# mariohsouto/ProxSDP.jl

Hardware: AMD Instinct MI355X
Metric: PDHG iterations/sec at target rank ~ sqrt(n), Max-Cut SDP n=4000 (tol 1e-4 options) (higher is better)
Workload: dtype f64

## Files before the change

### include/proxsdp_hip.h

```cpp
#ifndef PROXSDP_HIP_H
#define PROXSDP_HIP_H

#include <stdint.h>

#ifdef __cplusplus
extern "C" {
#endif

#define PROXSDP_HIP_ABI_VERSION 10

#define PROXSDP_E_INVALID  (-1)
#define PROXSDP_E_HIP      (-2)
#define PROXSDP_E_NOMEM    (-3)
#define PROXSDP_E_UNSUPP   (-4)
#define PROXSDP_E_INTERNAL (-5)
#define PROXSDP_E_COMM_ABORTED (-6)

#define PROXSDP_STATUS_NOT_CALLED       0
#define PROXSDP_STATUS_OPTIMAL          1
#define PROXSDP_STATUS_TIME_LIMIT       2
#define PROXSDP_STATUS_ITERATION_LIMIT  3
#define PROXSDP_STATUS_INFEAS_OR_UNBND  4
#define PROXSDP_STATUS_DUAL_INFEASIBLE  5
#define PROXSDP_STATUS_INFEASIBLE       6
// ... 29 lines not shown
    const double* M_dense;
    int32_t M_dense_on_device;
    int32_t reserved1;
    int64_t n_coupling;
    const int64_t* coupling_rows;
    const int32_t* coupling_owned;
    int (*reduce_vec_fn)(void* ctx, double* buf, int64_t len, int32_t on_device);
    int32_t reduce_vec_on_device;
    int32_t reserved2;
    void* nccl_comm;
    int64_t reserved3;
} proxsdp_problem;

typedef struct proxsdp_options {
    int64_t struct_size;
    int32_t log_verbose;  int32_t log_freq;
    int32_t timer_verbose; int32_t timer_file; int32_t disable_julia_logger;
    int32_t warn_on_limit; int32_t extended_log; int32_t extended_log2; int32_t log_repeat_header;
    int32_t pad0;
    double  time_limit;
    double tol_gap, tol_feasibility, tol_feasibility_dual, tol_primal, tol_dual, tol_psd, tol_soc;
    int32_t check_dual_feas; int32_t check_dual_feas_freq;
    double  max_obj; int32_t min_iter_max_obj; int32_t pad1;
    int32_t min_iter_time_infeas; int32_t pad2;
    double infeas_gap_tol, infeas_limit_gap_tol, infeas_stable_gap_tol,
           infeas_feasibility_tol, infeas_stable_feasibility_tol;
    int32_t certificate_search; int32_t pad3;
    double certificate_obj_tol, certificate_fail_tol;
    double min_beta, max_beta, initial_beta;
    double initial_adapt_level, adapt_decay; int32_t adapt_window; int32_t pad4;
    int32_t convergence_window; int32_t convergence_check;
    int64_t max_iter; int64_t min_iter; int64_t divergence_min_update;
    int64_t max_iter_lp; int64_t max_iter_conic; int64_t max_iter_local;
    int32_t advanced_initialization; int32_t line_search_flag;
    int32_t max_linsearch_steps; int32_t pad5;
    double delta, initial_theta, linsearch_decay;
    int32_t full_eig_decomp; int32_t max_target_rank_krylov_eigs;
    int32_t min_size_krylov_eigs; int32_t warm_start_eig;
    int32_t rank_increment; int32_t rank_increment_factor;
    int32_t eigsolver; int32_t eigsolver_min_lanczos; int64_t eigsolver_resid_seed;
    double  arpack_tol; int32_t arpack_resid_init; int32_t arpack_reset_resid; int64_t arpack_max_iter;
    int32_t krylovkit_reset_resid; int32_t krylovkit_resid_init;
    double  krylovkit_tol; int32_t krylovkit_max_iter; int32_t krylovkit_eager; int32_t krylovkit_verbose;
    int32_t reduce_rank; int32_t rank_slack; int32_t pad6;
    int64_t full_eig_freq; int64_t full_eig_len;
    int32_t equilibration; int32_t equilibration_iters;
    double  equilibration_lb, equilibration_ub, equilibration_limit;
    int32_t equilibration_force; int32_t approx_norm;
    int32_t device_id;
    int32_t trace_capacity;
    int32_t profile_symv_every;
    int32_t support_path;
    int32_t lanczos_operator;
    int32_t initial_target_rank;
    int32_t full_eig_lanczos;
    int32_t lanczos_cycle_kernel;
    int32_t lanczos_warm_start;
    int32_t reconstruct_mfma;
    int32_t small_block_batch;
    int32_t full_eig_sign;
    int32_t psd_sign_engine;
    int32_t full_eig_lanczos_verify;
    double  full_eig_lanczos_posres;
    int32_t full_eig_lanczos_kdim10;
    int32_t sign_small_tile_max;
    int32_t host_eig_threads;
    int32_t block_threads;
    int32_t host_eig_merge;
    int32_t block_batch;
    int32_t rocsolver_warmup;
    int32_t debug_fail_iteration;
    int32_t host_wait_spin;
    int32_t sign_start_row;
    int32_t general_batch;
    int32_t full_eig_lanczos_certify;
    int32_t host_merge_threads;
    int32_t reserved_i[1];
    double  full_eig_lanczos_tol;
    double  reserved_d[1];
    int32_t equilibration_reference_aliasing;
    int32_t reserved_i3[2];
    int32_t block_batch_groups;
    int32_t lanczos_wide_krylov;
    int32_t reserved_i2[7];
    double  full_eig_lanczos_warm_pow;
    double  reserved_d2[3];
} proxsdp_options;

#define PROXSDP_TRACE_COLS 14

typedef struct proxsdp_stats {
    int64_t lanczos_matvecs;
    int64_t lanczos_restarts;
    int64_t lanczos_calls;
    int64_t full_eigs;
    int64_t krylov_fallbacks;
    int64_t linesearch_trials;
    int64_t symv_launches;
    int64_t symv_profiled;
    double  symv_profiled_ms;
    double  symv_bytes;
    double  algorithmic_bytes;
    double  init_time;
    double  loop_time;
    double  exit_time;
    double  t_primal, t_psd, t_linesearch, t_residual;
    int64_t dense_passes;
    double  dense_ms;
    int64_t fop_projections;
    int64_t exit_matvecs;
    double  host_eig_time;
    int64_t host_eigs;
    int64_t device_eigs;
    int64_t batched_small_eigs;
    int64_t mfma_reconstructions;
    int64_t orth_profiled;
    double  orth_profiled_ms;
    double  full_eig_solver_ms;
    double  full_eig_recon_ms;
    int64_t cycle_launches;
    int64_t full_eigs_lanczos;
    int64_t cycle_steps;
    double  cycle_ms;
    int64_t warm_starts;
    int64_t full_eigs_sign;
    int64_t sign_products;
    int64_t sign_engine_projections;
    int64_t sign_engine_rejected;
    int64_t sign_engine_checks;
    int64_t sign_engine_mismatches;
    int64_t full_eigs_lanczos_checks;
    int64_t full_eigs_lanczos_mismatches;
    int64_t batched_block_steps;
    int64_t rccl_reductions;
    int64_t batched_profiled_blocks;
    int64_t host_eig_merges;
    double  host_eig_overlap_time;
    int64_t sign_short_pass;
    int64_t sign_short_fail;
    int64_t full_eigs_lanczos_certified;
    int64_t full_eigs_lanczos_cert_failed;
    int64_t cert_matvecs;
    int64_t dense_truncated_projections;
    int64_t wide_krylov_projections;
    int64_t reserved_s[4];
    int64_t dense_setup_passes;
    int64_t dense_sigma_steps;
} proxsdp_stats;
#define PROXSDP_STATS_SHARDED_GENERAL_ITERATIONS 0

typedef struct proxsdp_result {
    int32_t status;
    int32_t certificate_found;
    int32_t primal_feasible_user_tol;
    int32_t dual_feasible_user_tol;
    int32_t result_count;
    int32_t final_rank;
    int64_t iter;
    double  primal_residual;
    double  dual_residual;
    double  objval, dual_objval, gap, time;
    double  dual_feasibility;
    double* primal;
    double* dual_cone;
    double* dual_eq;
    double* dual_in;
    double* slack_eq;
    double* slack_in;
    double* trace;
    int64_t trace_rows;
    char    status_string[256];
    proxsdp_stats stats;
} proxsdp_result;

#define PROXSDP_STATE_NHIST 7
typedef struct proxsdp_state {
    int64_t struct_size;
    int64_t iteration;
    int64_t n, Q, n_psd;
    int64_t hist_len;
    double* x;
    double* y;
    double* Mty;
    double* Mx;
    int64_t* target_rank;
    int64_t* current_rank;
    double* min_eig;
    double* hist;
    double scal[16];
    int64_t ints[8];
} proxsdp_state;

int  proxsdp_hip_abi_version(void);
void proxsdp_hip_default_options(proxsdp_options* opt);
int  proxsdp_hip_set_option(proxsdp_options* opt, const char* name, double value);
int  proxsdp_hip_get_option(const proxsdp_options* opt, const char* name, double* value);
int  proxsdp_hip_solve(const proxsdp_problem* prob, const proxsdp_options* opt,
                       proxsdp_result* res);
int  proxsdp_hip_solve_ex(const proxsdp_problem* prob, const proxsdp_options* opt, proxsdp_result* res,
                          const proxsdp_state* resume, proxsdp_state* capture);
const char* proxsdp_hip_last_error(void);
int  proxsdp_hip_device_count(void);

int  proxsdp_hip_solve_sharded(const proxsdp_problem* prob, const proxsdp_options* opt,
                               int32_t n_shards, const int32_t* device_ids,
                               const int32_t* psd_owner, const int32_t* soc_owner, const int32_t* free_owner,
                               proxsdp_result* res, proxsdp_stats* shard_stats);

#define PROXSDP_FACTOR_NONE 0
#define PROXSDP_FACTOR_RITZ 1
#define PROXSDP_FACTOR_EIG  2
typedef struct proxsdp_psd_factors {
    int64_t struct_size;
    int64_t n_psd;
    const int64_t* cap;
    const int64_t* vec_ptr;
    const int64_t* val_ptr;
    double*  vectors;
    double*  values;
    int64_t* rank;
    int64_t* rank_found;
    int32_t* source;
    double*  resid;
    double*  xnorm;
} proxsdp_psd_factors;
int  proxsdp_hip_solve_factored(const proxsdp_problem* prob, const proxsdp_options* opt, proxsdp_result* res,
                                proxsdp_psd_factors* fac);

typedef struct proxsdp_start {
    int64_t struct_size;
    const double* primal;
    const double* dual_eq;
// ... 54 lines not shown
int proxsdp_hip_dual_trial(const double* y, const double* Mx, const double* Mx_old, const double* bh,
                           int64_t p, int64_t Q, double bt, double theta, double* y_out, double* ynorm2);

int proxsdp_hip_residuals(const double* x, const double* x_old, const double* Mty, const double* Mty_old,
                          const double* c, double tau, int64_t n,
                          const double* y, const double* y_old, const double* Mx, const double* Mx_old,
                          const double* bh, int64_t p, int64_t Q, double sigma, double* out);

typedef struct {
    int64_t struct_size;
    int64_t p;
    const double* bh; const double* y; const double* Mx; const double* Mx_old;
    const double* x; const double* x_old; const double* Mty_old;
    const double* roww;
    double xold_coef, tau_update;
    int32_t support, nc, plain, c0;
    double tau[3], theta[3], bt[3], sigma[3];
    double tau_re, sigma_re;
    double* y_out;
    double* Mty_out;
    double* scal;
    double* scal_re;
    int32_t* supp_out;
    double* x_upd; double* xsave; double* esv;
    int64_t ns;
    int32_t gq, gx;
} proxsdp_trial_batch;
int proxsdp_hip_trial_batch(const proxsdp_csc* M, int32_t index_base, const double* c, proxsdp_trial_batch* t);

int proxsdp_hip_cone_tail(const double* x, int64_t n, const int64_t* soc_off, const int32_t* soc_len, int32_t nsoc,
                          const int64_t* one_off, int32_t n_one, double* x_soc, double* gap_in, double* gap_out,
                          double* x_clamp, double* min_eig);

typedef struct {
    int64_t struct_size;
    int32_t n, tile, epilogue, use_dsc;
    const double* P; const double* Q; const double* Y;
    double ca, cb, cc;
    double dsc[3];
    const double* xold;
    const uint32_t* mask; int64_t mask_words, mask_off;
    double sentinel;
    double* T;
    double* part;
    double* xp;
    double* respart;
    int32_t ld, grid;
} proxsdp_sym_product;
int proxsdp_hip_sym_product(proxsdp_sym_product* t);

int proxsdp_hip_sign_unpack(const double* packed, int64_t n, double sentinel, double* A, double* sc);

int proxsdp_hip_dense_scaling(const proxsdp_problem* prob, const proxsdp_options* opt,
                              double* E, double* D, double* frob, double* sigma_max, int32_t* equilibrated);

int proxsdp_hip_coupling_sum(const double* parts, int32_t n_shards, int64_t len, const int64_t* rows,
                             const double* v_in, int64_t n, double* v_out);

typedef struct proxsdp_shard {
    int64_t struct_size;
    int64_t n, p, m, nnz_A, nnz_G, n_coupling, n_psd, len_psd, n_soc, len_soc, len_eig;
    int64_t* vars; int64_t* rows_eq; int64_t* rows_in;
    int64_t* coupling_rows; int32_t* coupling_owned;
    int64_t* A_colptr; int64_t* A_rowval; double* A_nzval;
    int64_t* G_colptr; int64_t* G_rowval; double* G_nzval;
    double* b; double* h; double* c;
    int64_t* psd_ids; int64_t* psd_ptr; int64_t* psd_idx;
    int64_t* soc_ids; int64_t* soc_ptr; int64_t* soc_idx;
    double* eig_resid;
} proxsdp_shard;
int proxsdp_host_split_shard(const proxsdp_problem* prob, int32_t n_shards, const int32_t* psd_owner,
                             const int32_t* soc_owner, const int32_t* free_owner, int32_t shard, proxsdp_shard* out);
int proxsdp_host_group_reduce(int32_t n_shards, int32_t rounds, int32_t nsum, int32_t nmax, const double* records,
                              int32_t leave_shard, int32_t leave_after, double timeout_s,
                              double* out, int32_t* rounds_done, int32_t* failed);
int proxsdp_host_symeig(int32_t k, double* a, double* d);
int proxsdp_host_symeig_threads(int32_t k, double* a, double* d, int32_t threads);
int proxsdp_host_symeig_arrow(int32_t K, int32_t m, const double* D, const double* f,
                              const double* al, const double* be, double* U, double* d);
int proxsdp_host_symeig_split(int32_t K, int32_t m, int32_t k1, const double* D, const double* f,
                              const double* al, const double* be, double* U, double* d, int32_t* info);
int proxsdp_host_symeig_split_threads(int32_t K, int32_t m, int32_t k1, const double* D, const double* f,
                                      const double* al, const double* be, int32_t threads, double* U, double* d, int32_t* info);
int proxsdp_host_start_vector(int64_t n, int64_t seed, int32_t init, double* out);
int proxsdp_host_preprocess(const proxsdp_problem* prob, int64_t* order, int64_t* var_ordering,
                            double* c_scaled, double* frobenius_norm_M);
int proxsdp_host_equilibrate_rowsums(const double* rowsums, int64_t Q, int64_t n, const proxsdp_options* opt,
                                     double* E, double* d);

#ifdef __cplusplus
}
#endif
#endif
```

### proxsdp.jl_amd/binding.py

```python
import ctypes as C
import os
import pathlib
import re

import numpy as np
import scipy.sparse as sp

_HERE = pathlib.Path(__file__).resolve().parent
LIB_PATH = _HERE / "libproxsdp_hip.so"
HEADER_PATH = _HERE.parent / "include" / "proxsdp_hip.h"

TRACE_COLS = 14
TRACE_NAMES = ("iter", "prim_obj", "dual_obj", "gap", "feas", "prim_res", "dual_res",
               "primal_step", "beta", "theta", "target_rank", "trials", "elapsed", "matvecs")


class LibraryNotBuilt(RuntimeError):
    pass


class ProxSDPHipError(RuntimeError):
    def __init__(self, code, msg):
        super().__init__(f"libproxsdp_hip error {code}: {msg}")
        self.code = code


i32, i64, f64 = C.c_int32, C.c_int64, C.c_double
pi64 = C.POINTER(C.c_int64)
pf64 = C.POINTER(C.c_double)


class CSC(C.Structure):
    _fields_ = [("nrows", i64), ("ncols", i64), ("colptr", pi64), ("rowval", pi64), ("nzval", pf64)]


class Problem(C.Structure):
    _fields_ = [("n", i64), ("p", i64), ("m", i64), ("A", CSC), ("G", CSC),
                ("b", pf64), ("h", pf64), ("c", pf64),
                ("n_psd", i64), ("psd_ptr", pi64), ("psd_idx", pi64),
                ("n_soc", i64), ("soc_ptr", pi64), ("soc_idx", pi64),
                ("index_base", i32), ("reserved0", i32), ("eig_resid", pf64),
                ("reduce_ctx", C.c_void_p), ("reduce_fn", C.c_void_p),
                ("M_dense", C.c_void_p), ("M_dense_on_device", i32), ("reserved1", i32),
                ("n_coupling", i64), ("coupling_rows", pi64), ("coupling_owned", C.POINTER(i32)),
                ("reduce_vec_fn", C.c_void_p), ("reduce_vec_on_device", i32), ("reserved2", i32),
                ("nccl_comm", C.c_void_p), ("reserved3", i64)]


REDUCE_FN = C.CFUNCTYPE(C.c_int, C.c_void_p, pf64, i32, pf64, i32)
REDUCE_VEC_FN = C.CFUNCTYPE(C.c_int, C.c_void_p, C.c_void_p, i64, i32)


def _opt_fields():
    F = []
    a = lambda name, t: F.append((name, t))
    a("struct_size", i64)
    for nme in ("log_verbose", "log_freq", "timer_verbose", "timer_file", "disable_julia_logger",
                "warn_on_limit", "extended_log", "extended_log2", "log_repeat_header", "pad0"):
        a(nme, i32)
    a("time_limit", f64)
    for nme in ("tol_gap", "tol_feasibility", "tol_feasibility_dual", "tol_primal", "tol_dual",
                "tol_psd", "tol_soc"):
        a(nme, f64)
    a("check_dual_feas", i32); a("check_dual_feas_freq", i32)
    a("max_obj", f64); a("min_iter_max_obj", i32); a("pad1", i32)
    a("min_iter_time_infeas", i32); a("pad2", i32)
    for nme in ("infeas_gap_tol", "infeas_limit_gap_tol", "infeas_stable_gap_tol",
                "infeas_feasibility_tol", "infeas_stable_feasibility_tol"):
        a(nme, f64)
    a("certificate_search", i32); a("pad3", i32)
    a("certificate_obj_tol", f64); a("certificate_fail_tol", f64)
    a("min_beta", f64); a("max_beta", f64); a("initial_beta", f64)
    a("initial_adapt_level", f64); a("adapt_decay", f64); a("adapt_window", i32); a("pad4", i32)
    a("convergence_window", i32); a("convergence_check", i32)
    for nme in ("max_iter", "min_iter", "divergence_min_update", "max_iter_lp", "max_iter_conic",
                "max_iter_local"):
        a(nme, i64)
    a("advanced_initialization", i32); a("line_search_flag", i32)
    a("max_linsearch_steps", i32); a("pad5", i32)
    a("delta", f64); a("initial_theta", f64); a("linsearch_decay", f64)
    a("full_eig_decomp", i32); a("max_target_rank_krylov_eigs", i32)
    a("min_size_krylov_eigs", i32); a("warm_start_eig", i32)
    a("rank_increment", i32); a("rank_increment_factor", i32)
    a("eigsolver", i32); a("eigsolver_min_lanczos", i32); a("eigsolver_resid_seed", i64)
    a("arpack_tol", f64); a("arpack_resid_init", i32); a("arpack_reset_resid", i32); a("arpack_max_iter", i64)
    a("krylovkit_reset_resid", i32); a("krylovkit_resid_init", i32)
    a("krylovkit_tol", f64); a("krylovkit_max_iter", i32); a("krylovkit_eager", i32); a("krylovkit_verbose", i32)
    a("reduce_rank", i32); a("rank_slack", i32); a("pad6", i32)
    a("full_eig_freq", i64); a("full_eig_len", i64)
    a("equilibration", i32); a("equilibration_iters", i32)
    a("equilibration_lb", f64); a("equilibration_ub", f64); a("equilibration_limit", f64)
    a("equilibration_force", i32); a("approx_norm", i32)
    a("device_id", i32); a("trace_capacity", i32); a("profile_symv_every", i32); a("support_path", i32)
    a("lanczos_operator", i32); a("initial_target_rank", i32)
    a("full_eig_lanczos", i32); a("lanczos_cycle_kernel", i32); a("lanczos_warm_start", i32)
    a("reconstruct_mfma", i32); a("small_block_batch", i32); a("full_eig_sign", i32); a("psd_sign_engine", i32)
    a("full_eig_lanczos_verify", i32); a("full_eig_lanczos_posres", f64); a("full_eig_lanczos_kdim10", i32)
    a("sign_small_tile_max", i32); a("host_eig_threads", i32); a("block_threads", i32)
    a("host_eig_merge", i32); a("block_batch", i32); a("rocsolver_warmup", i32); a("debug_fail_iteration", i32); a("host_wait_spin", i32)
    a("sign_start_row", i32); a("general_batch", i32); a("full_eig_lanczos_certify", i32); a("host_merge_threads", i32); a("reserved_i", i32 * 1)
    a("full_eig_lanczos_tol", f64); a("reserved_d", f64 * 1)
    a("equilibration_reference_aliasing", i32); a("reserved_i3", i32 * 2)
    a("block_batch_groups", i32); a("lanczos_wide_krylov", i32); a("reserved_i2", i32 * 7); a("full_eig_lanczos_warm_pow", f64); a("reserved_d2", f64 * 3)
    return F


class Options(C.Structure):
    _fields_ = _opt_fields()


class Stats(C.Structure):
    _fields_ = [("lanczos_matvecs", i64), ("lanczos_restarts", i64), ("lanczos_calls", i64),
                ("full_eigs", i64), ("krylov_fallbacks", i64), ("linesearch_trials", i64),
                ("symv_launches", i64), ("symv_profiled", i64), ("symv_profiled_ms", f64),
                ("symv_bytes", f64), ("algorithmic_bytes", f64), ("init_time", f64),
                ("loop_time", f64), ("exit_time", f64), ("t_primal", f64), ("t_psd", f64),
                ("t_linesearch", f64), ("t_residual", f64), ("dense_passes", i64), ("dense_ms", f64), ("fop_projections", i64), ("exit_matvecs", i64),
                ("host_eig_time", f64), ("host_eigs", i64), ("device_eigs", i64), ("batched_small_eigs", i64),
                ("mfma_reconstructions", i64), ("orth_profiled", i64), ("orth_profiled_ms", f64),
                ("full_eig_solver_ms", f64), ("full_eig_recon_ms", f64), ("cycle_launches", i64),
                ("full_eigs_lanczos", i64), ("cycle_steps", i64), ("cycle_ms", f64), ("warm_starts", i64),
                ("full_eigs_sign", i64), ("sign_products", i64),
                ("sign_engine_projections", i64), ("sign_engine_rejected", i64),
                ("sign_engine_checks", i64), ("sign_engine_mismatches", i64),
                ("full_eigs_lanczos_checks", i64), ("full_eigs_lanczos_mismatches", i64),
                ("batched_block_steps", i64), ("rccl_reductions", i64),
                ("batched_profiled_blocks", i64), ("host_eig_merges", i64),
                ("host_eig_overlap_time", f64), ("sign_short_pass", i64), ("sign_short_fail", i64),
                ("full_eigs_lanczos_certified", i64), ("full_eigs_lanczos_cert_failed", i64), ("cert_matvecs", i64),
                ("dense_truncated_projections", i64), ("wide_krylov_projections", i64), ("reserved_s", i64 * 4),
                ("dense_setup_passes", i64), ("dense_sigma_steps", i64)]


class Result(C.Structure):
    _fields_ = [("status", i32), ("certificate_found", i32), ("primal_feasible_user_tol", i32),
                ("dual_feasible_user_tol", i32), ("result_count", i32), ("final_rank", i32),
                ("iter", i64), ("primal_residual", f64), ("dual_residual", f64),
                ("objval", f64), ("dual_objval", f64), ("gap", f64), ("time", f64),
                ("dual_feasibility", f64),
                ("primal", pf64), ("dual_cone", pf64), ("dual_eq", pf64), ("dual_in", pf64),
                ("slack_eq", pf64), ("slack_in", pf64), ("trace", pf64), ("trace_rows", i64),
                ("status_string", C.c_char * 256), ("stats", Stats)]


STATS_RESERVED_SLOTS = {"sharded_general_iterations": 0}

STATE_NHIST = 7
STATE_HIST_NAMES = ("dual_gap", "prim_obj", "dual_obj", "feasibility", "primal_residual", "dual_residual", "comb_residual")
STATE_SCAL_NAMES = ("primal_step", "primal_step_old", "dual_step", "beta", "theta", "adapt_level",
                    "equa_feasibility", "ineq_feasibility", "dual_feasibility")


class State(C.Structure):
    _fields_ = [("struct_size", i64), ("iteration", i64), ("n", i64), ("Q", i64), ("n_psd", i64), ("hist_len", i64),
                ("x", pf64), ("y", pf64), ("Mty", pf64), ("Mx", pf64),
                ("target_rank", pi64), ("current_rank", pi64), ("min_eig", pf64), ("hist", pf64),
                ("scal", f64 * 16), ("ints", i64 * 8)]


class ShardIO(C.Structure):
    _fields_ = ([("struct_size", i64)] +
                [(k, i64) for k in ("n", "p", "m", "nnz_A", "nnz_G", "n_coupling", "n_psd", "len_psd", "n_soc", "len_soc", "len_eig")] +
                [("vars", pi64), ("rows_eq", pi64), ("rows_in", pi64), ("coupling_rows", pi64), ("coupling_owned", C.POINTER(i32)),
                 ("A_colptr", pi64), ("A_rowval", pi64), ("A_nzval", pf64), ("G_colptr", pi64), ("G_rowval", pi64), ("G_nzval", pf64),
                 ("b", pf64), ("h", pf64), ("c", pf64),
                 ("psd_ids", pi64), ("psd_ptr", pi64), ("psd_idx", pi64), ("soc_ids", pi64), ("soc_ptr", pi64), ("soc_idx", pi64), ("eig_resid", pf64)])


class PsdFactors(C.Structure):
    _fields_ = [("struct_size", i64), ("n_psd", i64), ("cap", pi64), ("vec_ptr", pi64), ("val_ptr", pi64),
                ("vectors", pf64), ("values", pf64), ("rank", pi64), ("rank_found", pi64), ("source", C.POINTER(i32)),
                ("resid", pf64), ("xnorm", pf64)]


class Start(C.Structure):
    _fields_ = [("struct_size", i64), ("primal", pf64), ("dual_eq", pf64), ("dual_in", pf64), ("n_psd", i64),
                ("rank", pi64), ("vec_ptr", pi64), ("val_ptr", pi64), ("vectors", pf64), ("values", pf64),
                ("target_rank", pi64), ("primal_step", f64), ("beta", f64)]


FACTOR_NONE, FACTOR_RITZ, FACTOR_EIG = 0, 1, 2
FACTOR_SOURCE_NAMES = {FACTOR_NONE: "NONE", FACTOR_RITZ: "RITZ", FACTOR_EIG: "EIG"}


_lib = None


def header_symbols():
    txt = HEADER_PATH.read_text()
    txt = re.sub(r"/\*.*?\*/", "", txt, flags=re.S)
    return sorted(set(re.findall(r"\b(proxsdp_(?:hip|host)_\w+)\s*\(", txt)))


def lib():
    global _lib
    if _lib is not None:
        return _lib
    if not LIB_PATH.exists():
        raise LibraryNotBuilt(
            f"{LIB_PATH} is missing: run `python -c 'import __graft_entry__ as g; g.build()'` "
            "(or `make -C proxsdp.jl_amd/csrc`).  There is no CPU fallback.")
    import sys
    if "torch" in sys.modules:
        try:
            tc = sys.modules["torch"].cuda
            if tc.is_available():
                tc.init()
        except Exception:
            pass
    L = C.CDLL(str(LIB_PATH))
    L.proxsdp_hip_abi_version.restype = C.c_int
    L.proxsdp_hip_last_error.restype = C.c_char_p
    L.proxsdp_hip_default_options.argtypes = [C.POINTER(Options)]
    L.proxsdp_hip_default_options.restype = None
    L.proxsdp_hip_set_option.argtypes = [C.POINTER(Options), C.c_char_p, f64]
    L.proxsdp_hip_get_option.argtypes = [C.POINTER(Options), C.c_char_p, pf64]
    L.proxsdp_hip_solve.argtypes = [C.POINTER(Problem), C.POINTER(Options), C.POINTER(Result)]
    L.proxsdp_hip_solve_ex.argtypes = [C.POINTER(Problem), C.POINTER(Options), C.POINTER(Result),
                                       C.POINTER(State), C.POINTER(State)]
    L.proxsdp_hip_solve_factored.argtypes = [C.POINTER(Problem), C.POINTER(Options), C.POINTER(Result),
                                             C.POINTER(PsdFactors)]
    L.proxsdp_hip_solve_from.argtypes = [C.POINTER(Problem), C.POINTER(Options), C.POINTER(Result),
                                         C.POINTER(Start), C.POINTER(PsdFactors)]
    L.proxsdp_hip_start_point.argtypes = [C.POINTER(Problem), C.POINTER(Options), C.POINTER(Start), C.POINTER(State)]
    L.proxsdp_hip_factor_residual.argtypes = [pf64, i64, pf64, i64, pf64, i32, pf64, pf64]
    L.proxsdp_hip_factor_residual_kernel.argtypes = [pf64, i64, pf64, i64, pf64, i32, pf64, pf64, i32, pf64]
    L.proxsdp_hip_psd_project.argtypes = [pf64, i64, i32, i32, C.POINTER(Options), pf64, pf64,
                                          C.POINTER(i32), pf64, pi64, C.POINTER(i32), C.POINTER(i32)]
# ... 778 lines not shown
    if epi < 2:
        out["T"] = np.zeros((ld, ld), order="F")
        t.T = _p(out["T"])
    else:
        out["xp"] = np.zeros(N)
        t.xp = _p(out["xp"])
    if want_part or epi >= 2:
        part = np.zeros(cap)
        t.part = _p(part)
    if epi == 3:
        xo = _f(xold)
        mk = np.ascontiguousarray(mask, dtype=np.uint32)
        assert len(xo) == N
        t.xold, t.mask, t.mask_words, t.mask_off = _p(xo), _p(mk, C.POINTER(C.c_uint32)), len(mk), int(mask_off)
        resp = np.zeros(2 * cap)
        t.respart = _p(resp)
    _check(lib().proxsdp_hip_sym_product(C.byref(t)))
    assert t.ld == ld and t.grid <= cap
    out.update(ld=ld, grid=int(t.grid), part=part[:t.grid].copy() if (want_part or epi >= 2) else None)
    if epi == 3:
        out["respart"] = resp[:2 * t.grid].reshape(2, t.grid).copy()
    return out


def sign_unpack(packed, n, sentinel=SYM_SENTINEL):
    xin = _f(packed)
    assert len(xin) == n * (n + 1) // 2
    ld = 64 * ((n + 63) // 64)
    A = np.zeros((ld, ld), order="F")
    sc = np.zeros(16)
    _check(lib().proxsdp_hip_sign_unpack(_p(xin), n, float(sentinel), _p(A), _p(sc)))
    return A, sc


def dense_scaling(prob, options=None):
    M = _Marshalled(prob)
    Q = M.P.p + M.P.m
    E, D = np.zeros(max(Q, 1)), np.zeros(max(M.P.n, 1))
    fro, sig, eq = f64(), f64(), i32()
    _check(lib().proxsdp_hip_dense_scaling(C.byref(M.P), C.byref(options) if options is not None else None,
                                           _p(E), _p(D), C.byref(fro), C.byref(sig), C.byref(eq)))
    return E[:Q], D[:M.P.n], fro.value, sig.value, bool(eq.value)


def host_symeig(A, threads=-1):
    L = lib()
    a = np.asfortranarray(A, dtype=np.float64).copy(order="F")
    k = a.shape[0]
    d = np.zeros(k)
    _check(L.proxsdp_host_symeig_threads(k, a.ctypes.data_as(pf64), _p(d), threads))
    return d, a


def host_symeig_arrow(D, f, al, be):
    L = lib()
    D, f, al, be = _f(D), _f(f), _f(al), _f(be)
    K, m = len(al), len(D)
    U = np.zeros((K, K), order="F")
    d = np.zeros(K)
    L.proxsdp_host_symeig_arrow.argtypes = [i32, i32, pf64, pf64, pf64, pf64, pf64, pf64]
    _check(L.proxsdp_host_symeig_arrow(K, m, _p(D), _p(f), _p(al), _p(be), U.ctypes.data_as(pf64), _p(d)))
    return d, U


def host_start_vector(n, seed=1234, init=3):
    out = np.zeros(n)
    _check(lib().proxsdp_host_start_vector(n, seed, init, _p(out)))
    return out


def host_symeig_split(D, f, al, be, k1, threads=0):
    D = _f(D); f = _f(f); al = _f(al); be = _f(be)
    K, m = len(al), len(D)
    U = np.zeros((K, K))
    d = np.zeros(K)
    info = (i32 * 3)()
    L = lib()
    L.proxsdp_host_symeig_split_threads.argtypes = [i32, i32, i32, pf64, pf64, pf64, pf64, i32, pf64, pf64, C.POINTER(i32)]
    _check(L.proxsdp_host_symeig_split_threads(K, m, int(k1), _p(D) if m else None, _p(f) if m else None, _p(al), _p(be),
                                               int(threads), _p(U), _p(d), info))
    return d, U.T.copy(), dict(nondeflated=info[0], deflated=info[1], max_secular_iterations=info[2])


def host_preprocess(prob, index_base=0):
    M = _Marshalled(prob, index_base=index_base)
    n = prob.n
    order, inv = np.zeros(n, dtype=np.int64), np.zeros(n, dtype=np.int64)
    cs = np.zeros(n)
    fro = f64()
    _check(lib().proxsdp_host_preprocess(C.byref(M.P), _p(order, pi64), _p(inv, pi64), _p(cs), C.byref(fro)))
    return order, inv, cs, fro.value


def host_equilibrate_rowsums(rowsums, n, options=None):
    rs = _f(rowsums)
    E = np.zeros(max(len(rs), 1))
    d = f64()
    _check(lib().proxsdp_host_equilibrate_rowsums(_p(rs), len(rs), int(n), C.byref(options) if options is not None else None,
                                                  _p(E), C.byref(d)))
    return E[:len(rs)], d.value
```

### proxsdp.jl_amd/csrc/capi.hip

```cpp
#include <functional>
#include <memory>
#include <new>
#include <string>

#include "pdhg_loop.hip.hpp"
#include "projection.hip.hpp"
#include "shard_split.hpp"

namespace {
thread_local std::string g_last_error;

template <typename F>
int guarded(F&& f) {
    try {
        g_last_error.clear();
        return f();
    } catch (const std::bad_alloc&) {
        g_last_error = "out of memory";
        return PROXSDP_E_NOMEM;
    } catch (const proxsdp::HipError& e) {
        g_last_error = e.what();
        return PROXSDP_E_HIP;
    } catch (const std::invalid_argument& e) {
        g_last_error = e.what();
// ... 853 lines not shown
    return guarded([&]() -> int {
        if (n <= 0 || Q <= 0 || p < 0 || p > Q || !x || !x_old || !Mty || !Mty_old || !c || !y || !y_old || !Mx ||
            !Mx_old || !bh || !out) throw std::invalid_argument("invalid argument");
        Engine E(nullptr, 2, 2);
        hipStream_t st = E.S.stream;
        using proxsdp::DevBuf;
        const int gx = std::min(proxsdp::PSTRIDE, proxsdp::grid_for(n)), gq = std::min(proxsdp::PSTRIDE, proxsdp::grid_for(Q));
        DevBuf<double> dx(n), dxo(n), dm(n), dmo(n), dc(n), dy(Q), dyo(Q), d1(Q), d0(Q), dbh(Q);
        DevBuf<double> part((size_t)11 * proxsdp::PSTRIDE), sc(9);
        dx.upload(x, n, st); dxo.upload(x_old, n, st); dm.upload(Mty, n, st); dmo.upload(Mty_old, n, st); dc.upload(c, n, st);
        dy.upload(y, Q, st); dyo.upload(y_old, Q, st); d1.upload(Mx, Q, st); d0.upload(Mx_old, Q, st); dbh.upload(bh, Q, st);
        part.zero(st);
        proxsdp::dev::TrialBatch tb{};
        tb.nc = 1; tb.tau[0] = tau; tb.sigma[0] = sigma;
        hipLaunchKernelGGL(proxsdp::dev::k_residual_xy<false>, dim3(std::max(gx, gq), 1, 2), dim3(proxsdp::dev::TPB), 0, st,
                           (const double*)dx.p, (const int*)nullptr, (long long)n, (const double*)dxo.p, 1.0,
                           (const double*)dm.p, (long long)n, (const double*)dmo.p, (const double*)dc.p, gx,
                           (const double*)dy.p, (long long)Q, (const double*)dyo.p, (const double*)d1.p, (const double*)d0.p,
                           (const double*)dbh.p, (int)p, (int)Q, gq, tb, part.p, proxsdp::PSTRIDE, 0LL, (const double*)nullptr);
        hipLaunchKernelGGL(proxsdp::dev::k_combine_multi, dim3(3), dim3(proxsdp::dev::TPB), 0, st,
                           (const double*)(part.p + (size_t)2 * proxsdp::PSTRIDE), proxsdp::PSTRIDE, gx, 0x3ull, sc.p, 3,
                           (const double*)nullptr, 0, 0, (double*)nullptr);
        hipLaunchKernelGGL(proxsdp::dev::k_combine_multi, dim3(6), dim3(proxsdp::dev::TPB), 0, st,
                           (const double*)(part.p + (size_t)5 * proxsdp::PSTRIDE), proxsdp::PSTRIDE, gq, 0xFull, sc.p + 3, 6,
                           (const double*)nullptr, 0, 0, (double*)nullptr);
        sc.download(out, 9, st);
        PX_HIP(hipStreamSynchronize(st));
        return 0;
    });
}

int proxsdp_host_symeig(int32_t k, double* a, double* d) {
    return proxsdp_host_symeig_threads(k, a, d, -1);
}

int proxsdp_host_symeig_threads(int32_t k, double* a, double* d, int32_t threads) {
    if (k < 0 || !a || !d) { g_last_error = "invalid argument"; return PROXSDP_E_INVALID; }
    int rc = proxsdp::symeig_dense(k, a, d, false, threads);
    if (rc != 0) { g_last_error = "QL iteration did not converge"; return PROXSDP_E_INTERNAL; }
    return 0;
}

int proxsdp_host_symeig_arrow(int32_t K, int32_t m, const double* D, const double* f,
                              const double* al, const double* be, double* U, double* d) {
    if (K < 2 || m < 1 || m >= K || !D || !f || !al || !be || !U || !d) { g_last_error = "invalid argument"; return PROXSDP_E_INVALID; }
    const int n1 = m + 1;
    std::vector<double> Qa((size_t)n1 * n1, 0.0), da(n1), ea(n1);
    for (int j = 0; j < m; ++j) { Qa[(size_t)j * n1 + j] = D[j]; Qa[(size_t)j * n1 + m] = Qa[(size_t)m * n1 + j] = f[j]; }
    proxsdp::householder_tridiag(n1, Qa.data(), da.data(), ea.data());
    int rc = proxsdp::symeig_tridiag_from(K, m, Qa.data(), da.data(), ea.data(), al, be, U, d);
    if (rc != 0) { g_last_error = "QL iteration did not converge"; return PROXSDP_E_INTERNAL; }
    return 0;
}

int proxsdp_host_symeig_split(int32_t K, int32_t m, int32_t k1, const double* D, const double* f,
                              const double* al, const double* be, double* U, double* d, int32_t* info) {
    return proxsdp_host_symeig_split_threads(K, m, k1, D, f, al, be, 0, U, d, info);
}

int proxsdp_host_symeig_split_threads(int32_t K, int32_t m, int32_t k1, const double* D, const double* f,
                                      const double* al, const double* be, int32_t threads, double* U, double* d, int32_t* info) {
    return guarded([&]() -> int {
        if (K < 2 || m < 0 || m >= K || k1 < 1 || k1 >= K || !al || !be || !U || !d) throw std::invalid_argument("invalid argument");
        proxsdp::SplitEig S;
        std::unique_ptr<proxsdp::SpinPool> pool;
        proxsdp::ParFor par;
        struct Guard { proxsdp::SpinPool* p; ~Guard() { if (p) p->disarm(); } } guard{nullptr};
        if (threads > 0) {
            pool.reset(new proxsdp::SpinPool(std::min<int>(threads, 15)));
            pool->arm();
            guard.p = pool.get();
            par = [&pool](int n, const std::function<void(int)>& body) { pool->run(n, body); };
            S.M.par = &par;
            S.M.nchunk = std::min<int>(threads, 15) + 1;
        }
        if (S.first(k1, m, D, f, al, be) != 0 || S.second(K, al, be) != 0) throw std::invalid_argument("split eigensolver failed");
        std::vector<int> cols(K);
        for (int c = 0; c < K; ++c) { cols[c] = c; d[c] = S.M.evals[c]; }
        S.M.vectors(cols.data(), K, U);
        if (info) { info[0] = S.M.k; info[1] = (int)S.M.df.size(); info[2] = S.M.max_iter_seen; }
        return 0;
    });
}
int proxsdp_host_start_vector(int64_t n, int64_t seed, int32_t init, double* out) {
    if (n < 0 || !out) { g_last_error = "invalid argument"; return PROXSDP_E_INVALID; }
    proxsdp::start_vector(n, (uint64_t)seed, init, out);
    return 0;
}

int proxsdp_host_preprocess(const proxsdp_problem* prob, int64_t* order, int64_t* var_ordering,
                            double* c_scaled, double* frobenius_norm_M) {
    return guarded([&]() -> int {
        if (!prob) throw std::invalid_argument("NULL problem");
        proxsdp::Prep R = proxsdp::prepare(*prob, nullptr, prob->reduce_fn != nullptr || prob->nccl_comm != nullptr);
        for (int64_t i = 0; i < R.n; ++i) {
            if (order) order[i] = R.ord[i];
            if (var_ordering) var_ordering[i] = R.inv[i];
            if (c_scaled) c_scaled[i] = R.c[i];
        }
        if (frobenius_norm_M) *frobenius_norm_M = R.frob;
        return 0;
    });
}

int proxsdp_host_split_shard(const proxsdp_problem* prob, int32_t n_shards, const int32_t* psd_owner,
                             const int32_t* soc_owner, const int32_t* free_owner, int32_t shard, proxsdp_shard* out) {
    return guarded([&]() -> int {
        if (!prob || !out) throw std::invalid_argument("NULL problem or output");
        if (out->struct_size != (int64_t)sizeof(proxsdp_shard)) throw std::invalid_argument("proxsdp_shard.struct_size mismatch");
        const proxsdp::ShardPlan L = proxsdp::plan_shards(*prob, n_shards, psd_owner, soc_owner, free_owner);
        if (shard < 0 || shard >= n_shards) throw std::invalid_argument("shard outside 0 .. n_shards - 1");
        const proxsdp::ShardData S = proxsdp::split_shard(*prob, L, shard);
        out->n = (int64_t)S.vars.size(); out->p = (int64_t)S.rows_eq.size(); out->m = (int64_t)S.rows_in.size();
        out->nnz_A = (int64_t)S.A_rowval.size(); out->nnz_G = (int64_t)S.G_rowval.size();
        out->n_coupling = (int64_t)S.coup_rows.size();
        out->n_psd = (int64_t)S.psd_ids.size(); out->len_psd = (int64_t)S.psd_idx.size();
        out->n_soc = (int64_t)S.soc_ids.size(); out->len_soc = (int64_t)S.soc_idx.size();
        out->len_eig = (int64_t)S.eig_resid.size();
        auto put = [](const auto& v, auto* dst) { if (dst) std::copy(v.begin(), v.end(), dst); };
        put(S.vars, out->vars); put(S.rows_eq, out->rows_eq); put(S.rows_in, out->rows_in);
        put(S.coup_rows, out->coupling_rows); put(S.coup_owned, out->coupling_owned);
        put(S.A_colptr, out->A_colptr); put(S.A_rowval, out->A_rowval); put(S.A_nzval, out->A_nzval);
        put(S.G_colptr, out->G_colptr); put(S.G_rowval, out->G_rowval); put(S.G_nzval, out->G_nzval);
        put(S.b, out->b); put(S.h, out->h); put(S.c, out->c);
        put(S.psd_ids, out->psd_ids); put(S.psd_ptr, out->psd_ptr); put(S.psd_idx, out->psd_idx);
        put(S.soc_ids, out->soc_ids); put(S.soc_ptr, out->soc_ptr); put(S.soc_idx, out->soc_idx);
        put(S.eig_resid, out->eig_resid);
        return 0;
    });
}

int proxsdp_host_group_reduce(int32_t n_shards, int32_t rounds, int32_t nsum, int32_t nmax, const double* records,
                              int32_t leave_shard, int32_t leave_after, double timeout_s,
                              double* out, int32_t* rounds_done, int32_t* failed) {
    return guarded([&]() -> int {
        if (n_shards < 1 || n_shards > 256 || rounds < 0 || nsum < 0 || nmax < 0 || nsum + nmax < 1 || !records || !out ||
            !rounds_done || !failed || leave_shard >= n_shards)
            throw std::invalid_argument("invalid argument");
        const size_t w = (size_t)nsum + (size_t)nmax;
        proxsdp::ShardGroup group(n_shards, timeout_s);
        auto body = [&](int s) {
            rounds_done[s] = 0; failed[s] = 0;
            try {
                for (int k = 0; k < rounds; ++k) {
                    if (s == leave_shard && k == leave_after) break;
                    const double* rec = records + ((size_t)k * n_shards + s) * w;
                    std::vector<double> sums(rec, rec + nsum), maxs(rec + nsum, rec + w);
                    group.reduce(s, sums, maxs);
                    double* o = out + ((size_t)s * rounds + k) * w;
                    std::copy(sums.begin(), sums.end(), o);
                    std::copy(maxs.begin(), maxs.end(), o + nsum);
                    rounds_done[s] = k + 1;
                }
            } catch (...) { failed[s] = 1; }
            group.leave();
        };
        run_shard_threads(n_shards, group, body);
        return 0;
    });
}

int proxsdp_host_equilibrate_rowsums(const double* rowsums, int64_t Q, int64_t n, const proxsdp_options* opt,
                                     double* E, double* d) {
    return guarded([&]() -> int {
        if (Q <= 0 || n <= 0 || !rowsums || !E || !d) throw std::invalid_argument("invalid argument");
        const proxsdp_options o = Engine::fix(opt);
// ... 25 lines not shown
```

### proxsdp.jl_amd/csrc/host_eig_merge.hpp

```cpp
#pragma once
#include <algorithm>
#include <cmath>
#include <functional>
#include <limits>
#include <vector>
#if defined(__x86_64__)
#include <immintrin.h>
#endif

namespace proxsdp {

#if defined(__x86_64__)
__attribute__((target("avx2,fma")))
static inline void rank1_panel_8x4(const double* Qf, int K, const int* qcol, int kk, int row, const double* w0,
                                   const double* w1, const double* w2, const double* w3, double* u0, double* u1,
                                   double* u2, double* u3) {
    __m256d a00 = _mm256_setzero_pd(), a10 = a00, a01 = a00, a11 = a00, a02 = a00, a12 = a00, a03 = a00, a13 = a00;
    for (int jj = 0; jj < kk; ++jj) {
        const double* qc = Qf + (size_t)qcol[jj] * K + row;
        const __m256d q0 = _mm256_loadu_pd(qc), q1 = _mm256_loadu_pd(qc + 4);
        __m256d w = _mm256_broadcast_sd(w0 + jj);
        a00 = _mm256_fmadd_pd(q0, w, a00); a10 = _mm256_fmadd_pd(q1, w, a10);
        w = _mm256_broadcast_sd(w1 + jj);
        a01 = _mm256_fmadd_pd(q0, w, a01); a11 = _mm256_fmadd_pd(q1, w, a11);
        w = _mm256_broadcast_sd(w2 + jj);
        a02 = _mm256_fmadd_pd(q0, w, a02); a12 = _mm256_fmadd_pd(q1, w, a12);
        w = _mm256_broadcast_sd(w3 + jj);
        a03 = _mm256_fmadd_pd(q0, w, a03); a13 = _mm256_fmadd_pd(q1, w, a13);
    }
    if (u0) { _mm256_storeu_pd(u0, a00); _mm256_storeu_pd(u0 + 4, a10); }
    if (u1) { _mm256_storeu_pd(u1, a01); _mm256_storeu_pd(u1 + 4, a11); }
    if (u2) { _mm256_storeu_pd(u2, a02); _mm256_storeu_pd(u2 + 4, a12); }
    if (u3) { _mm256_storeu_pd(u3, a03); _mm256_storeu_pd(u3 + 4, a13); }
}
#endif

using ParFor = std::function<void(int, const std::function<void(int)>&)>;

struct Rank1Merge {
    const ParFor* par = nullptr;
    int nchunk = 4;
    int K = 0, k1 = 0, k2 = 0, k = 0;
    double rho = 0.0;
    std::vector<double> Qf;
    std::vector<double> d, z;
    std::vector<char> ctype;
    std::vector<int> nd, df;
    std::vector<double> dn, zn;
    std::vector<double> lam;
    std::vector<double> delta;
    std::vector<double> S;
    std::vector<double> evals;
    std::vector<int> src;
    int max_iter_seen = 0;

    inline void eval(int org, double tau, int isplit, double& psi, double& dpsi, double& phi, double& dphi) const {
        const double dorg = dn[org];
        double a = 0.0, da = 0.0, b = 0.0, db = 0.0;
        for (int j = 0; j <= isplit; ++j) {
            const double dl = (dn[j] - dorg) - tau;
            const double t = zn[j] / dl;
            a += zn[j] * t; da += t * t;
        }
        for (int j = isplit + 1; j < k; ++j) {
            const double dl = (dn[j] - dorg) - tau;
            const double t = zn[j] / dl;
            b += zn[j] * t; db += t * t;
        }
        psi = rho * a; dpsi = rho * da; phi = rho * b; dphi = rho * db;
    }

    void solve_root(int i, int& org_out, double& tau_out, int& iters_out) const {
        const double eps = 2.220446049250313e-16;
        iters_out = 0;
        if (k == 1) { org_out = 0; tau_out = rho * zn[0] * zn[0]; return; }
        const bool last = (i == k - 1);
        const int ia = last ? k - 2 : i, ib = ia + 1;
        const int isplit = ia;
        double lo, hi;
        int org;
        double psi, dpsi, phi, dphi;
        if (!last) {
            const double gap = dn[i + 1] - dn[i];
            eval(i, 0.5 * gap, isplit, psi, dpsi, phi, dphi);
            const double fmid = 1.0 + psi + phi;
            if (fmid >= 0.0) { org = i; lo = 0.0; hi = 0.5 * gap; }
            else { org = i + 1; lo = -0.5 * gap; hi = 0.0; }
        } else {
            double zz = 0.0;
            for (int j = 0; j < k; ++j) zz += zn[j] * zn[j];
            org = k - 1; lo = 0.0; hi = rho * zz;
        }
        double tau = 0.5 * (lo + hi);
        double f = 0.0;
        int it = 0;
        for (; it < 80; ++it) {
            if (!(tau > lo && tau < hi)) tau = 0.5 * (lo + hi);
            if (tau == lo || tau == hi) break;
            eval(org, tau, isplit, psi, dpsi, phi, dphi);
            f = 1.0 + psi + phi;
            const double erretm = 8.0 * (std::fabs(psi) + std::fabs(phi)) + 2.0 + std::fabs(tau) * (dpsi + dphi);
            if (std::fabs(f) <= eps * erretm) break;
            if (f < 0.0) lo = tau; else hi = tau;
            if (hi - lo <= 2.0 * eps * std::max(std::fabs(lo), std::fabs(hi))) { tau = 0.5 * (lo + hi); break; }
            const double Da = (dn[ia] - dn[org]) - tau, Db = (dn[ib] - dn[org]) - tau;
            const double s = dpsi * Da * Da, Sb = dphi * Db * Db;
            const double c = f - dpsi * Da - dphi * Db;
            const double bq = c * (Da + Db) + s + Sb;
            const double w = Da * Db * f;
            double eta;
            if (c == 0.0) {
                eta = (bq != 0.0) ? w / bq : 0.0;
            } else {
                double disc = bq * bq - 4.0 * c * w;
                if (disc < 0.0) disc = 0.0;
                const double sq = std::sqrt(disc);
                const double q = (bq >= 0.0) ? 0.5 * (bq + sq) : 0.5 * (bq - sq);
                const double e1 = (q != 0.0) ? w / q : 0.0;
                const double e2 = q / c;
                const double t1 = tau + e1, t2 = tau + e2;
                const bool in1 = (t1 > lo && t1 < hi), in2 = (t2 > lo && t2 < hi);
                if (in1 && in2) eta = (std::fabs(e1) <= std::fabs(e2)) ? e1 : e2;
                else if (in1) eta = e1;
                else if (in2) eta = e2;
                else eta = 0.5 * (lo + hi) - tau;
            }
            double tn = tau + eta;
            if (!(tn > lo && tn < hi) || !(tn == tn)) tn = 0.5 * (lo + hi);
            if (tn == tau) break;
            tau = tn;
        }
        iters_out = it;
        org_out = org; tau_out = tau;
    }

    void build(int k1_, int k2_, const double* Q1, const double* d1, const double* Q2, const double* d2, double beta) {
        const double eps = 2.220446049250313e-16;
        k1 = k1_; k2 = k2_; K = k1 + k2;
        const double sgn = beta < 0.0 ? -1.0 : 1.0;
        rho = 2.0 * std::fabs(beta);
        const double isq2 = 0.70710678118654752440;
        d.assign(K, 0.0); z.assign(K, 0.0); ctype.assign(K, 0);
        Qf.assign((size_t)K * K, 0.0);
        {
            int a = 0, b = 0;
            for (int p = 0; p < K; ++p) {
                const bool takeA = (b >= k2) || (a < k1 && d1[a] <= d2[b]);
                double* col = Qf.data() + (size_t)p * K;
                if (takeA) {
                    d[p] = d1[a]; z[p] = Q1[(size_t)a * k1 + (k1 - 1)] * isq2; ctype[p] = 1;
                    for (int r = 0; r < k1; ++r) col[r] = Q1[(size_t)a * k1 + r];
                    ++a;
                } else {
                    d[p] = d2[b]; z[p] = sgn * Q2[(size_t)b * k2] * isq2; ctype[p] = 2;
                    for (int r = 0; r < k2; ++r) col[k1 + r] = Q2[(size_t)b * k2 + r];
                    ++b;
                }
            }
        }
        double zmax = 0.0, dmax = 0.0;
        for (int p = 0; p < K; ++p) { zmax = std::max(zmax, std::fabs(z[p])); dmax = std::max(dmax, std::fabs(d[p])); }
        const double tol = 8.0 * eps * std::max(dmax, zmax);
        nd.clear(); df.clear();
        if (rho * zmax <= tol) {
            for (int p = 0; p < K; ++p) df.push_back(p);
        } else {
            int pj = -1;
            for (int j = 0; j < K; ++j) {
                if (rho * std::fabs(z[j]) <= tol) { df.push_back(j); continue; }
                if (pj < 0) { pj = j; continue; }
                double s = z[pj], c = z[j];
                const double tau = std::sqrt(c * c + s * s);
                const double t = d[j] - d[pj];
                c /= tau; s = -s / tau;
                if (std::fabs(t * c * s) <= tol) {
                    z[j] = tau; z[pj] = 0.0;
                    double* __restrict__ x = Qf.data() + (size_t)pj * K;
                    double* __restrict__ y = Qf.data() + (size_t)j * K;
                    for (int r = 0; r < K; ++r) {
                        const double xr = x[r], yr = y[r];
                        x[r] = c * xr + s * yr;
                        y[r] = c * yr - s * xr;
                    }
                    const double tt = d[pj] * c * c + d[j] * s * s;
                    d[j] = d[pj] * s * s + d[j] * c * c;
                    d[pj] = tt;
                    if (ctype[pj] != ctype[j]) ctype[pj] = ctype[j] = 3;
                    df.push_back(pj);
                    pj = j;
                } else {
                    nd.push_back(pj);
                    pj = j;
                }
            }
            if (pj >= 0) nd.push_back(pj);
        }
        k = (int)nd.size();
        dn.resize(k); zn.resize(k);
        for (int j = 0; j < k; ++j) { dn[j] = d[nd[j]]; zn[j] = z[nd[j]]; }
        for (int j = 1; j < k; ++j)
            if (!(dn[j] > dn[j - 1])) dn[j] = std::nextafter(dn[j - 1], 1e300);
        lam.assign(k, 0.0);
        delta.assign((size_t)k * k, 0.0);
        max_iter_seen = 0;
        const int nc = (par != nullptr && k >= 32) ? std::max(1, nchunk) : 1;
        auto chunks = [&](const std::function<void(int, int)>& body) {
            if (nc == 1) { body(0, k); return; }
            const std::function<void(int)> one = [&](int c) { body((int)((long long)k * c / nc), (int)((long long)k * (c + 1) / nc)); };
            (*par)(nc, one);
        };
        std::vector<int> iters(std::max(k, 1), 0);
        chunks([&](int lo, int hi) {
            for (int i = lo; i < hi; ++i) {
                int org; double tau;
                solve_root(i, org, tau, iters[i]);
                lam[i] = dn[org] + tau;
                double* dl = delta.data() + (size_t)i * k;
                for (int j = 0; j < k; ++j) dl[j] = (dn[j] - dn[org]) - tau;
                if (dl[i] >= 0.0) dl[i] = -std::numeric_limits<double>::min();
                if (i + 1 < k && dl[i + 1] <= 0.0) dl[i + 1] = std::numeric_limits<double>::min();
            }
        });
        for (int i = 0; i < k; ++i) max_iter_seen = std::max(max_iter_seen, iters[i]);
        std::vector<double> zhat(k, 0.0);
        chunks([&](int lo, int hi) {
            for (int j = lo; j < hi; ++j) {
                double prod = -delta[(size_t)(k - 1) * k + j];
                for (int i = 0; i < j; ++i) prod *= delta[(size_t)i * k + j] / (dn[j] - dn[i]);
                for (int i = j; i < k - 1; ++i) prod *= delta[(size_t)i * k + j] / (dn[j] - dn[i + 1]);
                const double v = std::sqrt(std::fabs(prod) / rho);
                zhat[j] = zn[j] < 0.0 ? -v : v;
            }
        });
        S.assign((size_t)k * k, 0.0);
        chunks([&](int lo, int hi) {
            for (int i = lo; i < hi; ++i) {
                double* s = S.data() + (size_t)i * k;
                const double* dl = delta.data() + (size_t)i * k;
                double nn = 0.0;
                for (int j = 0; j < k; ++j) { s[j] = zhat[j] / dl[j]; nn += s[j] * s[j]; }
                const double inv = 1.0 / std::sqrt(nn);
                for (int j = 0; j < k; ++j) s[j] *= inv;
            }
        });
        std::vector<std::pair<double, int>> all;
        all.reserve(K);
        for (int i = 0; i < k; ++i) all.emplace_back(lam[i], i);
        for (int p : df) all.emplace_back(d[p], -(p + 1));
        std::stable_sort(all.begin(), all.end(), [](const std::pair<double, int>& a, const std::pair<double, int>& b) { return a.first < b.first; });
        evals.resize(K); src.resize(K);
        for (int c = 0; c < K; ++c) { evals[c] = all[c].first; src[c] = all[c].second; }
    }

    void row_of_vectors(int row, double* out) const {
        std::vector<double> qrow(k);
        for (int j = 0; j < k; ++j) qrow[j] = Qf[(size_t)nd[j] * K + row];
        for (int c = 0; c < K; ++c) {
            if (src[c] >= 0) {
                const double* s = S.data() + (size_t)src[c] * k;
                double a = 0.0;
                for (int j = 0; j < k; ++j) a += qrow[j] * s[j];
                out[c] = a;
            } else {
                out[c] = Qf[(size_t)(-(src[c] + 1)) * K + row];
            }
        }
    }

    void vectors(const int* cols, int ncols, double* U) const {
        std::vector<int> top, bot;
        for (int j = 0; j < k; ++j) {
            const char t = ctype[nd[j]];
            if (t == 1 || t == 3) top.push_back(j);
            if (t == 2 || t == 3) bot.push_back(j);
        }
        auto panel = [&](const std::vector<int>& idx, int r0, int nr) {
            const int kk = (int)idx.size();
            if (kk == 0 || nr <= 0) return;
            std::vector<int> qcol(kk);
            for (int jj = 0; jj < kk; ++jj) qcol[jj] = nd[idx[jj]];
            const int nblk = (ncols + 3) / 4;
            auto blocks = [&](int b0, int b1) {
            std::vector<double> wbuf((size_t)4 * kk);
            for (int c0 = 4 * b0; c0 < std::min(ncols, 4 * b1); c0 += 4) {
                const int cb = std::min(4, ncols - c0);
                double* u[4] = {nullptr, nullptr, nullptr, nullptr};
                for (int q = 0; q < 4; ++q) {
                    double* wq = wbuf.data() + (size_t)q * kk;
                    if (q < cb) {
                        u[q] = U + (size_t)(c0 + q) * K + r0;
                        const int sc = src[cols[c0 + q]];
                        if (sc >= 0) {
                            const double* sp = S.data() + (size_t)sc * k;
                            for (int jj = 0; jj < kk; ++jj) wq[jj] = sp[idx[jj]];
                        } else {
                            for (int jj = 0; jj < kk; ++jj) wq[jj] = 0.0;
                        }
                    } else {
                        for (int jj = 0; jj < kk; ++jj) wq[jj] = 0.0;
                    }
                }
                const double* w0 = wbuf.data(); const double* w1 = w0 + kk; const double* w2 = w1 + kk; const double* w3 = w2 + kk;
                int r = 0;
#if defined(__x86_64__)
                static const bool have_fma = __builtin_cpu_supports("avx2") && __builtin_cpu_supports("fma");
                for (; have_fma && r + 8 <= nr; r += 8)
                    rank1_panel_8x4(Qf.data(), K, qcol.data(), kk, r0 + r, w0, w1, w2, w3, u[0] ? u[0] + r : nullptr,
                                    u[1] ? u[1] + r : nullptr, u[2] ? u[2] + r : nullptr, u[3] ? u[3] + r : nullptr);
#endif
                for (; r < nr; ++r) {
                    double a0 = 0.0, a1 = 0.0, a2 = 0.0, a3 = 0.0;
                    for (int jj = 0; jj < kk; ++jj) {
                        const double qv = Qf[(size_t)qcol[jj] * K + r0 + r];
                        a0 += qv * w0[jj]; a1 += qv * w1[jj]; a2 += qv * w2[jj]; a3 += qv * w3[jj];
                    }
                    if (u[0]) u[0][r] = a0;
                    if (u[1]) u[1][r] = a1;
                    if (u[2]) u[2][r] = a2;
                    if (u[3]) u[3][r] = a3;
                }
            }
            };
            const int nc = (par != nullptr && nblk >= 8) ? std::max(1, nchunk) : 1;
            if (nc == 1) blocks(0, nblk);
            else {
                const std::function<void(int)> one = [&](int c) { blocks((int)((long long)nblk * c / nc), (int)((long long)nblk * (c + 1) / nc)); };
                (*par)(nc, one);
            }
        };
        std::fill(U, U + (size_t)K * ncols, 0.0);
        panel(top, 0, k1);
        panel(bot, k1, k2);
        for (int c = 0; c < ncols; ++c) {
            const int sc = src[cols[c]];
            if (sc >= 0) continue;
            const double* qc = Qf.data() + (size_t)(-(sc + 1)) * K;
            double* u = U + (size_t)c * K;
            for (int r = 0; r < K; ++r) u[r] = qc[r];
        }
    }
};

}
```

### proxsdp.jl_amd/csrc/host_util.hpp

```cpp
#pragma once
#include <atomic>
#include <chrono>
#include <cmath>
#include <condition_variable>
#include <cstdint>
#include <cstdlib>
#include <cstring>
#include <cstddef>
#include <functional>
#include <mutex>
#include <thread>
#include <vector>
#include <algorithm>
#if defined(__x86_64__)
#include <immintrin.h>
#endif
#include "../../include/proxsdp_hip.h"
#include "host_eig_merge.hpp"

namespace proxsdp {

inline uint64_t splitmix64(uint64_t z) {
    z += 0x9E3779B97F4A7C15ull;
    z = (z ^ (z >> 30)) * 0xBF58476D1CE4E5B9ull;
// ... 381 lines not shown
        if (gen_ == 0) gen_ = 1;
        const uint64_t g = gen_;
        ticket_.store(g << 32, std::memory_order_release);
        work(g);
        while (done_.load(std::memory_order_acquire) < n) {
#if defined(__x86_64__)
            _mm_pause();
#endif
        }
    }
private:
    void work(uint64_t g) {
        for (;;) {
            uint64_t t = ticket_.load(std::memory_order_acquire);
            if ((t >> 32) != g) return;
            const int i = (int)(t & 0xffffffffu);
            if (i >= njobs_.load(std::memory_order_relaxed)) return;
            if (!ticket_.compare_exchange_weak(t, t + 1, std::memory_order_acq_rel, std::memory_order_acquire)) continue;
            (*job_.load(std::memory_order_relaxed))(i);
            done_.fetch_add(1, std::memory_order_acq_rel);
        }
    }
    void loop() {
        uint64_t seen = 0;
        for (;;) {
            {
                std::unique_lock<std::mutex> lk(mu_);
                cv_.wait(lk, [&]() { return stop_.load() || armed_.load(std::memory_order_acquire); });
                if (stop_.load()) return;
            }
            while (armed_.load(std::memory_order_acquire) && !stop_.load(std::memory_order_relaxed)) {
                const uint64_t g = ticket_.load(std::memory_order_acquire) >> 32;
                if (g != seen) { seen = g; work(g); }
                else {
#if defined(__x86_64__)
                    _mm_pause();
#endif
                }
            }
        }
    }
    std::vector<std::thread> th_;
    std::mutex mu_;
    std::condition_variable cv_;
    std::atomic<bool> armed_{false}, stop_{false};
    uint64_t gen_ = 0;
    std::atomic<uint64_t> ticket_{0};
    std::atomic<int> done_{0}, njobs_{0};
    std::atomic<const std::function<void(int)>*> job_{nullptr};
};

struct SplitEig {
    Rank1Merge M;
    std::vector<double> Q1, d1, Q2, d2, e2;
    int k1 = 0, K = 0;
    double beta = 0.0;
    bool have_first = false;
    int first(int k1_, int m, const double* D, const double* f, const double* al, const double* be) {
        k1 = k1_; have_first = false;
        if (k1 < 1 || (m > 0 && k1 != m + 1)) return 1;
        beta = be[k1 - 1];
        if (!(beta == beta) || beta == 0.0) return 1;
        Q1.assign((size_t)k1 * k1, 0.0); d1.assign(k1, 0.0);
        int rc;
        if (m == 0) {
            for (int j = 0; j < k1; ++j) {
                Q1[(size_t)j * k1 + j] = al[j];
                if (j + 1 < k1) { Q1[(size_t)j * k1 + j + 1] = be[j]; Q1[(size_t)(j + 1) * k1 + j] = be[j]; }
            }
            Q1[(size_t)(k1 - 1) * k1 + (k1 - 1)] -= std::fabs(beta);
            rc = symeig_dense(k1, Q1.data(), d1.data(), true, 0);
        } else {
            for (int j = 0; j < m; ++j) {
                Q1[(size_t)j * k1 + j] = D[j];
                Q1[(size_t)j * k1 + m] = f[j]; Q1[(size_t)m * k1 + j] = f[j];
            }
            Q1[(size_t)m * k1 + m] = al[m] - std::fabs(beta);
            rc = symeig_dense(k1, Q1.data(), d1.data(), false, 0);
        }
        have_first = (rc == 0);
        return rc;
    }
    int second(int K_, const double* al, const double* be) {
        K = K_;
        const int k2 = K - k1;
        if (!have_first || k2 < 1) return 1;
        Q2.assign((size_t)k2 * k2, 0.0); d2.assign(k2, 0.0);
        for (int j = 0; j < k2; ++j) {
            Q2[(size_t)j * k2 + j] = al[k1 + j];
            if (j + 1 < k2) { Q2[(size_t)j * k2 + j + 1] = be[k1 + j]; Q2[(size_t)(j + 1) * k2 + j] = be[k1 + j]; }
        }
        Q2[0] -= std::fabs(beta);
        if (symeig_dense(k2, Q2.data(), d2.data(), true, 0) != 0) return 1;
        M.build(k1, k2, Q1.data(), d1.data(), Q2.data(), d2.data(), beta);
        return 0;
    }
};

enum OptType { OT_I32, OT_I64, OT_F64 };
struct OptEntry { const char* name; OptType type; size_t offset; };

#define PX_OPT(name, type) { #name, type, offsetof(proxsdp_options, name) }
inline const std::vector<OptEntry>& option_table() {
    static const std::vector<OptEntry> t = {
        PX_OPT(log_verbose, OT_I32), PX_OPT(log_freq, OT_I32), PX_OPT(timer_verbose, OT_I32),
        PX_OPT(timer_file, OT_I32), PX_OPT(disable_julia_logger, OT_I32), PX_OPT(warn_on_limit, OT_I32),
        PX_OPT(extended_log, OT_I32), PX_OPT(extended_log2, OT_I32), PX_OPT(log_repeat_header, OT_I32),
        PX_OPT(time_limit, OT_F64),
        PX_OPT(tol_gap, OT_F64), PX_OPT(tol_feasibility, OT_F64), PX_OPT(tol_feasibility_dual, OT_F64),
        PX_OPT(tol_primal, OT_F64), PX_OPT(tol_dual, OT_F64), PX_OPT(tol_psd, OT_F64), PX_OPT(tol_soc, OT_F64),
        PX_OPT(check_dual_feas, OT_I32), PX_OPT(check_dual_feas_freq, OT_I32),
        PX_OPT(max_obj, OT_F64), PX_OPT(min_iter_max_obj, OT_I32),
        PX_OPT(min_iter_time_infeas, OT_I32), PX_OPT(infeas_gap_tol, OT_F64),
        PX_OPT(infeas_limit_gap_tol, OT_F64), PX_OPT(infeas_stable_gap_tol, OT_F64),
        PX_OPT(infeas_feasibility_tol, OT_F64), PX_OPT(infeas_stable_feasibility_tol, OT_F64),
        PX_OPT(certificate_search, OT_I32), PX_OPT(certificate_obj_tol, OT_F64), PX_OPT(certificate_fail_tol, OT_F64),
        PX_OPT(min_beta, OT_F64), PX_OPT(max_beta, OT_F64), PX_OPT(initial_beta, OT_F64),
        PX_OPT(initial_adapt_level, OT_F64), PX_OPT(adapt_decay, OT_F64), PX_OPT(adapt_window, OT_I32),
        PX_OPT(convergence_window, OT_I32), PX_OPT(convergence_check, OT_I32),
        PX_OPT(max_iter, OT_I64), PX_OPT(min_iter, OT_I64), PX_OPT(divergence_min_update, OT_I64),
        PX_OPT(max_iter_lp, OT_I64), PX_OPT(max_iter_conic, OT_I64), PX_OPT(max_iter_local, OT_I64),
        PX_OPT(advanced_initialization, OT_I32), PX_OPT(line_search_flag, OT_I32),
        PX_OPT(max_linsearch_steps, OT_I32), PX_OPT(delta, OT_F64), PX_OPT(initial_theta, OT_F64),
        PX_OPT(linsearch_decay, OT_F64),
        PX_OPT(full_eig_decomp, OT_I32), PX_OPT(max_target_rank_krylov_eigs, OT_I32),
        PX_OPT(min_size_krylov_eigs, OT_I32), PX_OPT(warm_start_eig, OT_I32),
        PX_OPT(rank_increment, OT_I32), PX_OPT(rank_increment_factor, OT_I32),
        PX_OPT(eigsolver, OT_I32), PX_OPT(eigsolver_min_lanczos, OT_I32), PX_OPT(eigsolver_resid_seed, OT_I64),
        PX_OPT(arpack_tol, OT_F64), PX_OPT(arpack_resid_init, OT_I32), PX_OPT(arpack_reset_resid, OT_I32),
        PX_OPT(arpack_max_iter, OT_I64),
        PX_OPT(krylovkit_reset_resid, OT_I32), PX_OPT(krylovkit_resid_init, OT_I32),
        PX_OPT(krylovkit_tol, OT_F64), PX_OPT(krylovkit_max_iter, OT_I32), PX_OPT(krylovkit_eager, OT_I32),
        PX_OPT(krylovkit_verbose, OT_I32),
        PX_OPT(reduce_rank, OT_I32), PX_OPT(rank_slack, OT_I32),
        PX_OPT(full_eig_freq, OT_I64), PX_OPT(full_eig_len, OT_I64),
        PX_OPT(equilibration, OT_I32), PX_OPT(equilibration_iters, OT_I32),
        PX_OPT(equilibration_lb, OT_F64), PX_OPT(equilibration_ub, OT_F64), PX_OPT(equilibration_limit, OT_F64),
        PX_OPT(equilibration_force, OT_I32), PX_OPT(approx_norm, OT_I32),
        PX_OPT(device_id, OT_I32), PX_OPT(trace_capacity, OT_I32), PX_OPT(profile_symv_every, OT_I32),
        PX_OPT(support_path, OT_I32), PX_OPT(lanczos_operator, OT_I32), PX_OPT(initial_target_rank, OT_I32),
        PX_OPT(full_eig_lanczos, OT_I32), PX_OPT(lanczos_cycle_kernel, OT_I32), PX_OPT(lanczos_warm_start, OT_I32),
        PX_OPT(reconstruct_mfma, OT_I32), PX_OPT(small_block_batch, OT_I32), PX_OPT(full_eig_sign, OT_I32), PX_OPT(psd_sign_engine, OT_I32),
        PX_OPT(full_eig_lanczos_verify, OT_I32), PX_OPT(full_eig_lanczos_posres, OT_F64), PX_OPT(full_eig_lanczos_kdim10, OT_I32),
        PX_OPT(sign_small_tile_max, OT_I32), PX_OPT(host_eig_threads, OT_I32), PX_OPT(block_threads, OT_I32),
        PX_OPT(host_eig_merge, OT_I32), PX_OPT(block_batch, OT_I32),
        PX_OPT(rocsolver_warmup, OT_I32), PX_OPT(debug_fail_iteration, OT_I32), PX_OPT(host_wait_spin, OT_I32), PX_OPT(sign_start_row, OT_I32), PX_OPT(general_batch, OT_I32),
        PX_OPT(full_eig_lanczos_certify, OT_I32), PX_OPT(full_eig_lanczos_tol, OT_F64), PX_OPT(host_merge_threads, OT_I32),
        PX_OPT(equilibration_reference_aliasing, OT_I32), PX_OPT(block_batch_groups, OT_I32), PX_OPT(full_eig_lanczos_warm_pow, OT_F64),
        PX_OPT(lanczos_wide_krylov, OT_I32),
    };
    return t;
}
#undef PX_OPT

inline void default_options(proxsdp_options* o) {
    std::memset(o, 0, sizeof(*o));
    o->struct_size = (int64_t)sizeof(*o);
    o->log_verbose = 0; o->log_freq = 1000; o->disable_julia_logger = 1;
    o->time_limit = 360000.0;
    o->tol_gap = 1e-4; o->tol_feasibility = 1e-4; o->tol_feasibility_dual = 1e-4;
    o->tol_primal = 1e-4; o->tol_dual = 1e-4; o->tol_psd = 1e-7; o->tol_soc = 1e-7;
    o->check_dual_feas = 0; o->check_dual_feas_freq = 1000;
    o->max_obj = 1e20; o->min_iter_max_obj = 10;
    o->min_iter_time_infeas = 1000; o->infeas_gap_tol = 1e-4; o->infeas_limit_gap_tol = 1e-1;
    o->infeas_stable_gap_tol = 1e-4; o->infeas_feasibility_tol = 1e-4;
    o->infeas_stable_feasibility_tol = 1e-8;
    o->certificate_search = 1; o->certificate_obj_tol = 1e-1; o->certificate_fail_tol = 1e-8;
    o->min_beta = 1e-5; o->max_beta = 1e5; o->initial_beta = 1.0;
    o->initial_adapt_level = 0.9; o->adapt_decay = 0.8; o->adapt_window = 50;
    o->convergence_window = 200; o->convergence_check = 50;
    o->max_iter = 0; o->min_iter = 40; o->divergence_min_update = 50;
    o->max_iter_lp = 10000000; o->max_iter_conic = 1000000; o->max_iter_local = 0;
    o->advanced_initialization = 1; o->line_search_flag = 1; o->max_linsearch_steps = 5000;
    o->delta = 0.9999; o->initial_theta = 1.0; o->linsearch_decay = 0.75;
    o->full_eig_decomp = 0; o->max_target_rank_krylov_eigs = 16; o->min_size_krylov_eigs = 100;
    o->warm_start_eig = 1; o->rank_increment = 1; o->rank_increment_factor = 1;
    o->eigsolver = 2; o->eigsolver_min_lanczos = 25; o->eigsolver_resid_seed = 1234;
    o->arpack_tol = 1e-10; o->arpack_resid_init = 3; o->arpack_reset_resid = 1; o->arpack_max_iter = 10000;
    o->krylovkit_reset_resid = 0; o->krylovkit_resid_init = 3; o->krylovkit_tol = 1e-12;
    o->krylovkit_max_iter = 100; o->krylovkit_eager = 0; o->krylovkit_verbose = 0;
    o->reduce_rank = 0; o->rank_slack = 3; o->full_eig_freq = 10000000; o->full_eig_len = 0;
    o->equilibration = 0; o->equilibration_iters = 1000; o->equilibration_lb = -10.0;
    o->equilibration_ub = 10.0; o->equilibration_limit = 0.9; o->equilibration_force = 0;
    o->approx_norm = 1;
    o->device_id = 0; o->trace_capacity = 0; o->profile_symv_every = 0; o->support_path = -1;
    o->lanczos_operator = -1; o->initial_target_rank = 2;
    o->full_eig_lanczos = -1; o->lanczos_cycle_kernel = -1; o->lanczos_warm_start = 0; o->reconstruct_mfma = -1;
    o->small_block_batch = -1; o->full_eig_sign = -1; o->psd_sign_engine = -1;
    o->full_eig_lanczos_verify = -1; o->full_eig_lanczos_posres = 1e-6; o->full_eig_lanczos_kdim10 = 30;
    o->sign_small_tile_max = 3072; o->host_eig_threads = 0; o->block_threads = -1;
    o->host_eig_merge = -1; o->block_batch = -1; o->rocsolver_warmup = 0; o->host_wait_spin = -1; o->sign_start_row = -1; o->general_batch = -1;
    o->full_eig_lanczos_certify = -1; o->full_eig_lanczos_tol = 0.0; o->host_merge_threads = -1;
    o->equilibration_reference_aliasing = 1; o->block_batch_groups = -1; o->full_eig_lanczos_warm_pow = 1.0;
    o->lanczos_wide_krylov = 0;
}

inline int set_option(proxsdp_options* o, const char* name, double v) {
    for (const auto& e : option_table()) {
        if (std::strcmp(e.name, name) == 0) {
            char* base = reinterpret_cast<char*>(o) + e.offset;
            if (e.type == OT_I32) *reinterpret_cast<int32_t*>(base) = (int32_t)std::llround(v);
            else if (e.type == OT_I64) *reinterpret_cast<int64_t*>(base) = (int64_t)std::llround(v);
            else *reinterpret_cast<double*>(base) = v;
            return 0;
        }
    }
    return PROXSDP_E_INVALID;
}
inline int get_option(const proxsdp_options* o, const char* name, double* v) {
    for (const auto& e : option_table()) {
        if (std::strcmp(e.name, name) == 0) {
            const char* base = reinterpret_cast<const char*>(o) + e.offset;
            if (e.type == OT_I32) *v = (double)*reinterpret_cast<const int32_t*>(base);
            else if (e.type == OT_I64) *v = (double)*reinterpret_cast<const int64_t*>(base);
            else *v = *reinterpret_cast<const double*>(base);
            return 0;
        }
    }
    return PROXSDP_E_INVALID;
}

}
```

### proxsdp.jl_amd/csrc/solver.hip.hpp

```cpp
#pragma once
#include <hip/hip_runtime.h>
#include <hip/hip_ext.h>
#include <array>
#include <memory>
#include <mutex>
#include <condition_variable>
#include <functional>
#include <exception>
#include <rocblas/rocblas.h>
#include <rocsolver/rocsolver.h>

#include <algorithm>
#include <chrono>
#include <cmath>
#include <cstdio>
#include <cstdlib>
#include <cstring>
#include <stdexcept>
#include <string>
#include <thread>
#include <tuple>
#include <type_traits>
#include <utility>
#include <vector>
// ... 53 lines not shown
    void upload(const T* h, size_t count, hipStream_t s) {
        if (count) PX_HIP(hipMemcpyAsync(p, h, count * sizeof(T), hipMemcpyHostToDevice, s));
    }
    void download(T* h, size_t count, hipStream_t s) const {
        if (count) PX_HIP(hipMemcpyAsync(h, p, count * sizeof(T), hipMemcpyDeviceToHost, s));
    }
};

struct PinnedBuf {
    double* p = nullptr;
    PinnedBuf() = default;
    PinnedBuf(const PinnedBuf&) = delete;
    PinnedBuf& operator=(const PinnedBuf&) = delete;
    PinnedBuf(PinnedBuf&& o) noexcept : p(o.p) { o.p = nullptr; }
    PinnedBuf& operator=(PinnedBuf&& o) noexcept { if (this != &o) { release(); p = o.p; o.p = nullptr; } return *this; }
    ~PinnedBuf() { release(); }
    void alloc(size_t count, unsigned flags = hipHostMallocDefault) {
        release();
        if (hipHostMalloc((void**)&p, count * sizeof(double), flags) != hipSuccess) { p = nullptr; throw std::bad_alloc(); }
    }
    void release() { if (p) { (void)hipHostFree(p); p = nullptr; } }
};

template <typename H, typename Traits>
struct Owned {
    H h = nullptr;
    Owned() = default;
    Owned(const Owned&) = delete;
    Owned& operator=(const Owned&) = delete;
    Owned(Owned&& o) noexcept : h(o.h) { o.h = nullptr; }
    Owned& operator=(Owned&& o) noexcept { if (this != &o) { release(); h = o.h; o.h = nullptr; } return *this; }
    ~Owned() { release(); }
    void release() { if (h) { Traits::destroy(h); h = nullptr; } }
    operator H() const { return h; }
};
struct EventTraits { static void destroy(hipEvent_t e) { (void)hipEventDestroy(e); } };
struct StreamTraits { static void destroy(hipStream_t s) { (void)hipStreamDestroy(s); } };
struct BlasTraits { static void destroy(rocblas_handle b) { (void)rocblas_destroy_handle(b); } };
struct Event : Owned<hipEvent_t, EventTraits> {
    void create(unsigned flags = hipEventDefault) { if (!h) PX_HIP(hipEventCreateWithFlags(&h, flags)); }
};
struct Stream : Owned<hipStream_t, StreamTraits> {
    void create(unsigned flags = hipStreamDefault) { if (!h) PX_HIP(hipStreamCreateWithFlags(&h, flags)); }
};
struct BlasHandle : Owned<rocblas_handle, BlasTraits> {
    void create() { if (!h) PX_ROC(rocblas_create_handle(&h)); }
};

template <typename F>
inline double time_launches(hipStream_t s, int repeat, F&& launch) {
    Event a, b;
    a.create(); b.create();
    PX_HIP(hipEventRecord(a, s));
    for (int i = 0; i < repeat; ++i) launch();
    PX_HIP(hipEventRecord(b, s));
    PX_HIP(hipEventSynchronize(b));
    float t = 0.f;
    PX_HIP(hipEventElapsedTime(&t, a, b));
    return (double)t / repeat;
}

static inline double now_s() {
    return std::chrono::duration<double>(std::chrono::steady_clock::now().time_since_epoch()).count();
}
static inline int ceil_div(long long a, long long b) { return (int)((a + b - 1) / b); }
static inline int grid_for(long long n) {
    long long g = (n + dev::TPB - 1) / dev::TPB;
    return (int)std::max<long long>(1, std::min<long long>(g, 2048));
}
template <typename Query, typename GiveUp>
inline void poll_ready(Query query, GiveUp give_up) {
    for (unsigned spins = 0;; ++spins) {
        const hipError_t e = query();
        if (e == hipSuccess) return;
        if (e != hipErrorNotReady) PX_HIP(e);
        if ((spins & 0xfff) == 0xfff) give_up();
#if defined(__x86_64__)
        _mm_pause();
#endif
    }
}
}
#include "shard_comm.hip.hpp"
namespace proxsdp {

struct CircularVector {
    std::vector<double> v;
    int l = 0;
    void init(int len) { v.assign(len, 0.0); l = len; }
    double& at(long long i) { return v[(size_t)(((i - 1) % l + l) % l)]; }
    double max_abs_diff() const {
        double val = 0.0;
        for (int i = 0; i < l; ++i) val = std::max(val, std::fabs(v[i] - v[(i + l - 1) % l]));
        return val;
    }
};

struct EigEvents {
    std::vector<Event> e0, e1;
    size_t used = 0;
    std::pair<hipEvent_t, hipEvent_t> acquire() {
        if (used == e0.size()) {
            Event a, b;
            a.create(); b.create();
            e0.push_back(std::move(a)); e1.push_back(std::move(b));
        }
        ++used;
        return {e0[used - 1], e1[used - 1]};
    }
    void harvest(double& ms_sum, int64_t& count) {
        for (size_t s = 0; s < used; ++s) {
            float ms = 0.f;
            if (hipEventElapsedTime(&ms, e0[s], e1[s]) == hipSuccess) { ms_sum += ms; count++; }
        }
        used = 0;
    }
};

struct StreamRef {
    Stream main;
    static inline thread_local hipStream_t tl = nullptr;
    operator hipStream_t() const { return tl ? tl : main.h; }
};

struct LzRun {
    int nev = 0, krylovdim = 0, ld = 0;
    bool arpack = false, positive_part = false;
    double tol = 0.0, step_tol = 0.0;
    long long maxiter = 0;
    std::vector<double> T, Tw, D, U, f, al, be, Qa, da, ea;
    int howmany = 0, numiter = 1, converged = 0, K = 0, kfirst = 0, pos_count = -1, m_arrow = 0;
    bool pos_fail = false, presymv = false;
    double betaK = 0.0;
    const double* rec = nullptr;
    int rec_ld = 0;
    bool wide = false;
    SplitEig* splitp = nullptr;
    SplitEig& split_ref() { return *splitp; }
    bool split_ready = false;
    bool merge_active = false;
    std::vector<double> erow;
};

struct EigWork {
    int n = 0, nt = 0, npad = 0, nwg = 0, cap = 0, pld = 0;
    int64_t N = 0;
    DevBuf<double> V, Z;
    DevBuf<double> w, Ppart, hpart1, hpart2, hsum1, hred, U, lam, resid, Apart, arrow;
    DevBuf<double> resid2;
    int napart = 0;
    PinnedBuf arrow_host;
    const double* arrow_p = nullptr;
    DevBuf<double> rec;
    double* alphas_p = nullptr; double* betas_p = nullptr; dev::LanczosCtl* ctl_p = nullptr;
    PinnedBuf rec_pinned;
    double* rec_host = nullptr;
    static constexpr size_t REC_DOUBLES = 2 * dev::MAXK + sizeof(dev::LanczosCtl) / sizeof(double);
    static constexpr size_t USTAGE_DOUBLES = (size_t)dev::MAXK * dev::MAXK + 2 * dev::MAXK;
    size_t ustage_doubles = USTAGE_DOUBLES;
    bool wide = false;
    DevBuf<double> hpw1, hpw2, hsw1, hsw2, recw;
    PinnedBuf recw_pinned;
    dev::LanczosCtl* ctlw_p = nullptr;
    static constexpr size_t RECW_DOUBLES = 2 * dev::LZW_MAXK + sizeof(dev::LanczosCtl) / sizeof(double);
    DevBuf<double> A, D, E;
    DevBuf<rocblas_int> info;
    std::vector<double> resid_host;
    PinnedBuf Ustage[2];
    int ustage_next = 0;
    std::vector<double> vals;
    int count = 0, converged_eigs = 0, numiter = 0, prev_numiter = 1;
    bool converged = false;
    DevBuf<double> F, Flam, tpart, ebuf, apartf;
    DevBuf<int> ell_col, ell_sidx;
    DevBuf<int> wr_ptr, wr_row, wr_lo, wr_hi, ov_col, ov_sidx;
    dev::EllOverflow ov{};
    int ell_w = 0, F_first = 0, F_r = 0;
    bool fop_ok = false;
    bool have_factors = false;
    bool use_fop = false;
    struct XPrev {
        bool sparse = true;
        int last_npos = -1;
    } xprev;
    void forget_factors() { have_factors = false; xprev.sparse = false; use_fop = false; }
    bool ritz_ok = false;
    int ritz_first = 0, ritz_r = 0;
    PinnedBuf rec_early;
    SplitEig split;
    int batch_slot = 0;
    bool b1_defer = false;
    int b1_rot_K = 0;
    const double* b1_rot_U = nullptr;
    LzRun lzrun;
    struct LanczosFullEig {
        long long served = 0;
        bool disabled = false;
        int cert_fails = 0;
    } fel;
    DevBuf<double> warm_part;
    bool cye_pending = false;
    const double* esv = nullptr;
    proxsdp_stats lst{};
    long long mv_iter = 0, recon_r = 0;
    bool fe_pending = false;
    DevBuf<double> sgA, sgX, sgX2, sgY, sgQ, sg_part, sg_part2, sg_sc;
    PinnedBuf sg_host;
    int sg_ld = 0;
    int sg_npart = 0;
    int sg_row = -1, sg_ok = 16, sg_idle = 0, sg_hold = 0;
    bool sg_small = false;
    int sg_nt48 = 0;
    bool sg_pending = false;
    struct SignStandIn {
        double kry_ms = -1.0, sign_ms = -1.0;
        int streak = 0, backoff = 0;
        int verified_left = 0;
        bool disabled = false, check_pending = false;
    } sign;
    DevBuf<double> sg_cmp;
    DevBuf<double> sg_out;
    Stream stream;
    Event done;
    Stream side;
    Event ev_mid, ev_early;
    EigEvents ev, evo;
    Event fe[3];
    Event cye[2];
    Event sg_ev;
};
static_assert(std::is_nothrow_move_constructible<EigWork>::value, "eig.resize() moves workspaces");


static inline void count_matvecs(EigWork& W, long long c) {
    W.lst.symv_launches += c;
    W.lst.symv_bytes += (double)c * (8.0 * (double)W.N + 16.0 * (double)W.n);
}

static inline int lz_nch(int cols) { return (cols <= 64) ? 1 : (cols <= 128) ? 2 : (cols <= 192) ? 3 : 4; }
template <typename F>
static inline void with_nch(int cols, F&& f) {
    switch (lz_nch(cols)) {
        case 1: f(std::integral_constant<int, 1>{}); break;
        case 2: f(std::integral_constant<int, 2>{}); break;
        case 3: f(std::integral_constant<int, 3>{}); break;
        default: f(std::integral_constant<int, 4>{}); break;
    }
}

struct RotSink {
    struct Req { EigWork* W = nullptr; const double* V = nullptr; double* out = nullptr; int K = 0, ncols = 0, copy_src = -1,
                 copy_dst = 0, nextra = 0; bool valid = false; std::vector<double> data; };
    std::array<Req, dev::LZB_MAX> slot;
};

class Solver {
public:
    Solver(const proxsdp_problem& prob, const proxsdp_options& opt_in, proxsdp_result& res_out,
           ShardGroup* grp = nullptr, int grp_rank = 0)
        : opt(opt_in), res(res_out), time0(now_s()), P(prepare(prob, &opt_in, grp != nullptr || prob.reduce_fn != nullptr || prob.nccl_comm != nullptr)) {
        user_resid = prob.eig_resid;
        if (grp) comm.reset(new GroupComm(*grp, grp_rank, opt.host_wait_spin != 0));
        else if (prob.nccl_comm != nullptr) comm.reset(new RcclComm(prob.nccl_comm, st));
        else if (prob.reduce_fn != nullptr) comm.reset(new CallbackComm(prob));
        if (prob.n_coupling > 0) {
            if ((!prob.reduce_fn || !prob.reduce_vec_fn) && prob.nccl_comm == nullptr && grp == nullptr)
                throw std::invalid_argument("coupling rows need nccl_comm, or reduce_fn and reduce_vec_fn");
            if (!prob.coupling_rows || !prob.coupling_owned)
                throw std::invalid_argument("coupling rows need coupling_rows and coupling_owned");
            for (int64_t k = 0; k < prob.n_coupling; ++k) {
                const int64_t r = prob.coupling_rows[k];
                if (r < 0 || r >= prob.p + prob.m) throw std::invalid_argument("coupling row out of range");
// ... 8 lines not shown
    ~Solver() {
        if (warm.joinable()) warm.join();
        block_pool.reset();
    }
    void run();
    void check_run_options();
    void init_parameters();
    void reduce_global_constants();
    void start_host_helpers();
    void alloc_iterate_pairs();
    void alloc_iterate();
    void classify_blocks();
    void start_block_workers();
    void setup_small_batch();
    void setup_soc();
    bool initial_steps();
    enum class Loop { next, stop };
    void iterate(long long k);
    Loop after_iteration(long long k);
    void finish();
    enum class Cert { infeasible, dual_infeasible };
    bool declare(int reason, const std::string& str, Cert kind, bool at_limit = false);
    void cert_infeas();
    void cert_dual_infeas();
    void snapshot();
    void update_dual_feasibility(const std::vector<double>& cvec);
    double loop_t0 = 0;
    bool shard_general = false;

    void setup_device();
    void alloc_eigwork(EigWork& W, int n, int max_nev);
    void lanczos_start_vector(EigWork& W, const double* user);
    void lanczos(EigWork& W, const double* xp, int nev, bool positive_part = false);
    void lz_launch_step(EigWork& W, const double* xp, int k, int kfirst, double step_tol, bool& presymv);
    void lz_launch_finish(EigWork& W, int k, double tol, bool use_carry);
    void lz_launch_begin(EigWork& W, const double* start, dev::LanczosCtl* ctl);
    bool lanczos_certificate(EigWork& W, const double* xp, int npos, int msteps, double& theta_max, double& scale);
    void lanczos_batch(const std::vector<int>& blocks, const double* xbase, const std::vector<int>& nevs, int ctx_slot = 0);
    double dbg_batch[5] = {0, 0, 0, 0, 0};
    double dbg_lz[8] = {0, 0, 0, 0, 0, 0, 0, 0};
    static inline thread_local RotSink* rot_sink = nullptr;
    struct BatchCtx {
        DevBuf<double> U;
        PinnedBuf U_host, rec_host;
        std::unique_ptr<SpinPool> pool;
        Event ev;
    };
    std::vector<std::unique_ptr<BatchCtx>> batch_ctx;
    std::mutex batch_stats_mu;
    std::unique_ptr<SpinPool> merge_pool;
    ParFor merge_par;
    int merge_helpers() const { return opt.host_merge_threads < 0 ? 3 : std::min(15, (int)opt.host_merge_threads); }
    static constexpr size_t LZB_USTRIDE = 64 * 64 + 2 * dev::MAXK;
    void flush_rotations(RotSink& sink, BatchCtx& C);
    bool lz_init(EigWork& W, struct LzRun& R, int nev, bool positive_part);
    void lz_prepare_arrow(struct LzRun& R);
    bool lz_after_cycle(EigWork& W, struct LzRun& R, bool speculated);
    void lz_rayleigh(EigWork& W, struct LzRun& R, int K, double betaK, bool from_arrow, bool check_first);
    void lz_restart(EigWork& W, struct LzRun& R, int K, int keep, bool speculated);
    void lz_finish_run(EigWork& W, struct LzRun& R);
    void lanczos_eager(EigWork& W, const double* xp, int nev);
    void lzw_step(EigWork& W, const double* xp, int k, int kfirst, double step_tol, bool& presymv);
    void lz_merge_vectors(EigWork& W, struct LzRun& R, int ncols);
    bool lz_split_first(EigWork& W, struct LzRun& R, int k1);
    void full_eig_values(EigWork& W, const double* xp, double offscale, bool vectors, std::vector<double>& Dhost);
    void begin_full_eig_events(EigWork& W);
    void harvest_full_eig_events(EigWork& W);
    int block1_lds_cap = 0;
    DevBuf<long long> b1_dbg;
    bool block1_plan(const EigWork& W, int krylovdim, bool split_wanted) const;
    void launch_block1(EigWork& W, const double* xp, int kfirst, int krylovdim, double tol);
    bool sg48_ok = false;
    void launch_symv(EigWork& W, const double* xp, const double* v, bool use_ctl, dev::LanczosCtl* ctl = nullptr);
    void launch_symv_finish(EigWork& W, const double* xp, int kclose, double tol, bool use_carry);
    void launch_reconstruct(EigWork& W, const double* Z, int ldz, const double* lam, int r, double* xp_out,
                            const double* xp_old = nullptr, int blk = -1);
    proxsdp_psd_factors* factors_out = nullptr;
    DevBuf<double> fac_V, fac_lam, fac_part;
    void factor_residual(const double* xp, int n, const double* V, int ldv, const double* lam, int r,
                         double& resid2, double& xnorm2);
    void extract_factors(const std::vector<double>& x);
    void rotate(EigWork& W, int K, const std::vector<double>& U, int ldu, int ncols, double* out, int copy_src, int copy_dst,
                const double* extra, int nextra);

    void test_project(int idx, double* xp, int tr);
    void test_full_eig(const double* xin, double* xout) { current_rank.assign(1, 0); min_eig.assign(1, 0.0); full_eig_project(0, xin, xout, false); }
    long long test_rank() const { return current_rank.empty() ? 0 : current_rank[0]; }
    double test_min_eig() const { return min_eig.empty() ? 0.0 : min_eig[0]; }
    void test_spmv(bool transpose, const double* in, double* out);
    void test_trial_batch(proxsdp_trial_batch& t);
    void test_cone_tail(const double* x, int64_t n, const int64_t* so, const int32_t* sl, int nsoc,
                        const int64_t* oo, int none, double* x_soc, double* gap_in, double* gap_out,
                        double* x_clamp, double* mineig);
    void test_sym_product(proxsdp_sym_product& t);
    void test_sign_unpack(const double* packed, double sentinel, double* A, double* sc);

    bool debug = std::getenv("PROXSDP_HIP_DEBUG") != nullptr;
    proxsdp_options opt;
    proxsdp_result& res;
    double time0 = 0;
    Prep P;
    proxsdp_stats st{};
    const double* user_resid = nullptr;
    std::unique_ptr<ShardComm> comm;
    bool sharded() const { return comm != nullptr; }
    long long current_iteration() const { return iter; }
    std::exception_ptr shard_error;
    void reduce(std::vector<double>& sums, std::vector<double>& maxs) { if (comm) comm->reduce(stream, sums, maxs); }
    void reduce_vec_host(std::vector<double>& v) { if (!v.empty()) comm->reduce_vec_host(stream, v); }
    std::vector<int> coup_rows;
    std::vector<char> coup_owned;
    DevBuf<int> coup_rows_d;
    DevBuf<double> roww_d;
    void reduce_coupling(double* Mx_dev) {
        if (!coup_rows.empty()) comm->reduce_coupling(stream, Mx_dev, coup_rows_d.p, (int)coup_rows.size());
    }
    void wait_stream() {
        if (!comm || !comm->bounded_wait(stream)) wait_for_stream(stream, opt.host_wait_spin != 0);
    }
    const proxsdp_state* resume_state = nullptr;
    proxsdp_state* capture_state = nullptr;
    void check_state_shape(const proxsdp_state& s, const char* what) const;
    void apply_resume();
    void write_capture();
    const proxsdp_start* start = nullptr;
    proxsdp_state* start_out = nullptr;
    bool start_active = false;
    DevBuf<long long> start_ord_d;
    DevBuf<double> start_src_d, start_V, start_lam;
    void apply_start();
    void write_start_point();
    int ada_count = 0;
    void wait_event(hipEvent_t ev) {
        if (opt.host_wait_spin == 0) PX_HIP(hipEventSynchronize(ev));
        else poll_ready([&]() { return hipEventQuery(ev); }, []() {});
    }
    double g_n = 0, g_Q = 0, g_p = 0, g_m = 0, g_norm_b = 0, g_norm_h = 0, g_norm_c = 0, g_frob = 0;
    bool g_conic = false, g_not_converged_rank = false, g_any_below_full = false;
    double g_elapsed = 0;
    bool init_only = false;
    double sigma_max = 0.0;
    std::thread warm;
    std::mutex blas_mutex;
    std::unique_ptr<BlockPool> block_pool;
    bool parallel_blocks() const { return block_pool != nullptr; }
    void run_blocks(const std::vector<int>& blocks, const std::function<void(int)>& job);
    void merge_block_stats();
    void start_rocsolver_warmup();

private:
    DevBuf<double> xbuf[2], Mtybuf[2], ybuf[2], Mxbuf[2], c_d, bh_d, part, scal;
    DevBuf<int> csr_ptr, csr_col, csc_ptr, csc_row;
    DevBuf<double> csr_val, csc_val;
    DevBuf<long long> one_off, soc_off;
    DevBuf<int> soc_len;
    DevBuf<double> one_min, soc_gap_d;
    int xc = 0, mtyc = 0, yc = 0, mxc = 0;
    std::vector<int> one_blocks;
    std::vector<int> big_blocks;
    std::vector<int> small_blocks, large_blocks;
    DevBuf<long long> small_off;
    DevBuf<int> small_side, small_rank;
    PinnedBuf small_rank_host;
    int small_maxn = 0;
    int small_jacobi_max = 64;
    int small_sign_maxn = 0;
// ... 381 lines not shown
    count_matvecs(W, 1);
}

inline void Solver::lz_launch_finish(EigWork& W, int k, double tol, bool use_carry) {
    with_nch(k + 1, [&](auto nch) {
        hipLaunchKernelGGL(dev::k_lz_finish<decltype(nch)::value>, dim3(W.nt), dim3(dev::TPB), 0, stream,
                           (const double*)W.w.p, W.n, W.V.p, W.npad, k, (const double*)lz_hpart(W, k), W.pld,
                           (const double*)W.hsum1.p, W.alphas_p, W.betas_p, W.ctl_p, tol, use_carry ? 1 : 0, W.hred.p);
    });
}

inline void Solver::lz_launch_begin(EigWork& W, const double* start, dev::LanczosCtl* ctl) {
    hipLaunchKernelGGL(dev::k_lz_begin, dim3(ceil_div(W.npad, dev::TPB)), dim3(dev::TPB), 0, stream,
                       W.V.p, start, W.npad, ctl);
}

inline void Solver::launch_reconstruct(EigWork& W, const double* Z, int ldz, const double* lam, int r, double* xp_out,
                                       const double* xp_old, int blk) {
    const int ntile = 8 * ceil_div(W.nt * (W.nt + 1) / 2, 8);
    const bool mfma = opt.reconstruct_mfma == 1 || (opt.reconstruct_mfma < 0 && r >= 16);
    if (mfma) {
        W.lst.mfma_reconstructions++;
        if (use_support && xp_old != nullptr && blk >= 0)
            hipLaunchKernelGGL(dev::k_reconstruct_mfma<true>, dim3(ntile), dim3(dev::TPB), 0, stream,
                               Z, ldz, lam, r, W.n, xp_out, xp_old, mask_d.p, (long long)P.blocks[blk].off,
                               respart_d.p + tile_base[blk], rstride);
        else
            hipLaunchKernelGGL(dev::k_reconstruct_mfma<false>, dim3(ntile), dim3(dev::TPB), 0, stream,
                               Z, ldz, lam, r, W.n, xp_out, (const double*)nullptr, (const unsigned*)nullptr, 0LL,
                               (double*)nullptr, 0);
        return;
    }
    if (use_support && xp_old != nullptr && blk >= 0)
        hipLaunchKernelGGL(dev::k_reconstruct_packed<true>, dim3(ntile), dim3(dev::TPB), 0, stream,
                           Z, ldz, lam, r, W.n, xp_out, xp_old, mask_d.p, (long long)P.blocks[blk].off,
                           respart_d.p + tile_base[blk], rstride);
    else
        hipLaunchKernelGGL(dev::k_reconstruct_packed<false>, dim3(ntile), dim3(dev::TPB), 0, stream,
                           Z, ldz, lam, r, W.n, xp_out, (const double*)nullptr, (const unsigned*)nullptr, 0LL,
                           (double*)nullptr, 0);
}

inline void Solver::factor_residual(const double* xp, int n, const double* V, int ldv, const double* lam, int r,
                                    double& resid2, double& xnorm2) {
    const int nt = ceil_div(n, dev::TILE);
    const int tiles = nt * (nt + 1) / 2;
    if (fac_part.n < (size_t)2 * tiles) fac_part.alloc((size_t)2 * tiles);
    hipLaunchKernelGGL(dev::k_factor_residual, dim3(8 * ceil_div(tiles, 8)), dim3(dev::TPB), 0, stream,
                       xp, n, V, ldv, lam, r, fac_part.p);
    PX_HIP(hipGetLastError());
    std::vector<double> h((size_t)2 * tiles);
    fac_part.download(h.data(), h.size(), stream);
    PX_HIP(hipStreamSynchronize(stream));
    resid2 = 0.0; xnorm2 = 0.0;
    for (int t = 0; t < tiles; ++t) { resid2 += h[2 * t]; xnorm2 += h[2 * t + 1]; }
}

inline void Solver::rotate(EigWork& W, int K, const std::vector<double>& U, int ldu, int ncols,
                           double* out, int copy_src, int copy_dst, const double* extra, int nextra) {
    if (rot_sink != nullptr) {
        RotSink::Req& q = rot_sink->slot[W.batch_slot];
        q.W = &W; q.V = W.V.p; q.out = out; q.K = K; q.ncols = ncols; q.copy_src = copy_src; q.copy_dst = copy_dst;
        q.nextra = std::max(nextra, 0); q.valid = true;
        q.data.resize((size_t)K * std::max(ncols, 0) + (size_t)q.nextra);
        for (int c = 0; c < ncols; ++c)
            for (int j = 0; j < K; ++j) q.data[(size_t)c * K + j] = U[(size_t)c * ldu + j];
        for (int t = 0; t < q.nextra; ++t) q.data[(size_t)K * std::max(ncols, 0) + t] = extra[t];
        return;
    }
    double* tmp = W.Ustage[W.ustage_next].p;
    W.ustage_next ^= 1;
    if ((size_t)K * std::max(ncols, 1) + (size_t)std::max(nextra, 0) > W.ustage_doubles)
        throw std::logic_error("rotation staging buffer too small");
    for (int c = 0; c < ncols; ++c)
        for (int j = 0; j < K; ++j) tmp[(size_t)c * K + j] = U[(size_t)c * ldu + j];
    for (int q = 0; q < nextra; ++q) tmp[(size_t)K * ncols + q] = extra[q];
    if (W.b1_defer && nextra > 0 && K < 32 && copy_src == K && copy_dst == ncols && out == W.Z.p) {
        W.b1_rot_K = K; W.b1_rot_U = tmp;
        W.arrow_p = tmp + (size_t)K * ncols;
        return;
    }
    W.U.upload(tmp, (size_t)K * ncols + (size_t)std::max(nextra, 0), stream);
    if (nextra > 0) W.arrow_p = W.U.p + (size_t)K * ncols;
    if (W.lzrun.wide) {
        if (ncols > 0 || copy_src >= 0)
            hipLaunchKernelGGL(dev::k_lzw_rotate, dim3(W.nt, std::max(1, ceil_div(ncols, dev::LZW_RC))), dim3(dev::TPB), 0, stream,
                               (const double*)W.V.p, W.npad, K, (const double*)W.U.p, ncols, out, W.npad, copy_src, copy_dst);
        return;
    }
    {
        const int Kp = (K + 3) & ~3;
        const size_t lds_m = ((size_t)Kp * dev::RM_LDV + (size_t)dev::RM_CG * (Kp + 2)) * sizeof(double);
        if (K >= 32 && ncols >= 16 && (int)lds_m <= rotate_mfma_lds_cap) {
            hipLaunchKernelGGL(dev::k_lz_rotate_mfma, dim3(W.nt, ceil_div(ncols, dev::RM_CG)), dim3(dev::TPB), lds_m, stream,
                               (const double*)W.V.p, W.npad, K, (const double*)W.U.p, ncols, out, W.npad, copy_src, copy_dst);
            return;
        }
    }
    const int vbytes = K * (dev::LZ_ROWS + 1) * 8;
    const int maxcols = std::max(1, (rotate_lds_cap - vbytes) / (8 * K));
    int c0 = 0;
    do {
        const int cn = std::max(0, std::min(maxcols, ncols - c0));
        const bool last = (c0 + cn >= ncols);
        if (cn > 0 || (last && copy_src >= 0))
            hipLaunchKernelGGL(dev::k_lz_rotate, dim3(W.nt), dim3(dev::TPB), (size_t)K * cn * 8 + vbytes, stream,
                               W.V.p, W.npad, W.n, K, W.U.p + (size_t)c0 * K, K, cn,
                               out + (size_t)c0 * W.npad, W.npad, last ? copy_src : -1, copy_dst - c0);
        c0 += std::max(cn, 1);
    } while (c0 < ncols);
}

inline bool Solver::lz_init(EigWork& W, LzRun& R, int nev, bool positive_part) {
    R.nev = nev; R.positive_part = positive_part;
    W.b1_rot_K = 0; W.b1_rot_U = nullptr;
    R.arpack = (opt.eigsolver == 1);
    int krylovdim = krylov_dim(nev);
    if (positive_part) {
        const int mult10 = opt.full_eig_lanczos_kdim10 > 0 ? opt.full_eig_lanczos_kdim10 : 30;
        krylovdim = std::min(std::min(W.cap, dev::MAXK - 4) - 1, std::max(krylovdim, nev * mult10 / 10 + 8));
    }
    if (krylovdim + 1 > W.cap) throw std::invalid_argument("Lanczos workspace too small for the requested rank");
    R.krylovdim = krylovdim;
    R.wide = krylovdim > dev::LZ_KMAX;
    if (R.wide && !W.wide) throw std::logic_error("wide Lanczos: workspace has no wide records");
    R.rec = R.wide ? W.recw_pinned.p : W.rec_host;
    R.rec_ld = R.wide ? dev::LZW_MAXK : dev::MAXK;
    R.tol = R.arpack ? opt.arpack_tol : opt.krylovkit_tol;
    R.maxiter = R.arpack ? (long long)opt.arpack_max_iter : (long long)opt.krylovkit_max_iter;
    W.prev_numiter = std::max(W.numiter, 1);
    W.converged = false; W.count = 0; W.converged_eigs = 0; W.numiter = 0; W.vals.clear();
    W.lst.lanczos_calls++;
    if (R.arpack && (!(0 < nev && nev < W.n) || krylovdim > W.n)) return false;
    R.step_tol = R.arpack ? 0.0 : R.tol;
    R.ld = krylovdim + 1;
    R.T.assign((size_t)R.ld * R.ld, 0.0); R.D.assign(R.ld, 0.0); R.f.assign(R.ld, 0.0);
    R.al.assign(R.ld, 0.0); R.be.assign(R.ld, 0.0);
    R.howmany = nev; R.numiter = 1; R.converged = 0; R.K = 0; R.kfirst = 0; R.pos_count = -1;
    R.pos_fail = false; R.presymv = false; R.betaK = 0.0;
    R.split_ready = false; R.merge_active = false;
    R.splitp = &W.split;
    return true;
}

inline void Solver::lz_merge_vectors(EigWork& W, LzRun& R, int ncols) {
    const double t0 = now_s();
    const int K = R.K;
    std::vector<int> cols(std::max(ncols, 1));
    for (int c = 0; c < ncols; ++c) cols[c] = K - 1 - c;
    R.U.assign((size_t)K * std::max(ncols, 1), 0.0);
    if (ncols > 0) R.split_ref().M.vectors(cols.data(), ncols, R.U.data());
    W.lst.host_eig_time += now_s() - t0;
}

inline void Solver::lz_prepare_arrow(LzRun& R) {
    R.m_arrow = R.kfirst;
    if (R.m_arrow <= 0) return;
    const int n1 = R.m_arrow + 1, ld = R.ld;
    R.Qa.assign((size_t)n1 * n1, 0.0); R.da.assign(n1, 0.0); R.ea.assign(n1, 0.0);
    for (int j = 0; j < R.m_arrow; ++j) {
        R.Qa[(size_t)j * n1 + j] = R.T[(size_t)j * ld + j];
        R.Qa[(size_t)j * n1 + R.m_arrow] = R.Qa[(size_t)R.m_arrow * n1 + j] = R.T[(size_t)j * ld + R.m_arrow];
    }
    householder_tridiag(n1, R.Qa.data(), R.da.data(), R.ea.data());
}

inline bool Solver::lz_after_cycle(EigWork& W, LzRun& R, bool speculated) {
    const int krylovdim = R.krylovdim, ld = R.ld, kfirst = R.kfirst, nev = R.nev;
    const double tol = R.tol;
    std::vector<double>& T = R.T; std::vector<double>& D = R.D; std::vector<double>& f = R.f;
    std::vector<double>& al = R.al; std::vector<double>& be = R.be;
    dev::LanczosCtl hctl{};
    std::copy(R.rec, R.rec + krylovdim, al.begin());
    std::copy(R.rec + R.rec_ld, R.rec + R.rec_ld + krylovdim, be.begin());
    std::memcpy(&hctl, R.rec + 2 * R.rec_ld, sizeof(hctl));
    const int Kend = hctl.stop ? hctl.kstop : krylovdim;
    W.lst.lanczos_matvecs += (Kend - kfirst);
    count_matvecs(W, -(long long)(krylovdim - Kend));
    W.mv_iter += (Kend - kfirst);
    for (int k = kfirst; k < Kend; ++k) {
        T[(size_t)k * ld + k] = al[k];
        if (k + 1 < Kend) { T[(size_t)k * ld + k + 1] = be[k]; T[(size_t)(k + 1) * ld + k] = be[k]; }
    }
    const int K = R.K = Kend;
    const double betaK = R.betaK = be[K - 1];
    if (!(betaK == betaK)) {
        R.converged = 0; R.pos_fail = true; R.howmany = 0;
        return false;
    }
    if (betaK <= tol && K < R.howmany && !R.arpack) R.howmany = K;
    R.merge_active = false;
    if (K > 1 && R.split_ready && K == krylovdim) {
        const double te0 = now_s();
        if (R.split_ref().second(K, al.data(), be.data()) == 0) {
            R.erow.resize(K);
            R.split_ref().M.row_of_vectors(K - 1, R.erow.data());
            for (int c = 0; c < K; ++c) {
                D[c] = R.split_ref().M.evals[K - 1 - c];
                f[c] = betaK * R.erow[K - 1 - c];
            }
            R.merge_active = true;
            W.lst.host_eigs++; W.lst.host_eig_merges++;
        }
        W.lst.host_eig_time += now_s() - te0;
    }
    R.split_ready = false;
    if (!R.merge_active) lz_rayleigh(W, R, K, betaK, true, kfirst == 0);
    int converged = 0;
    if (!R.arpack) {
        double tol_c = tol;
        if (R.positive_part && opt.full_eig_lanczos_tol > 0.0)
            tol_c = std::max(tol, opt.full_eig_lanczos_tol * std::max(std::fabs(D[0]), std::fabs(D[K - 1])));
        while (converged < K && std::fabs(f[converged]) <= tol_c) ++converged;
    } else {
        const double eps23 = std::pow(2.220446049250313e-16 / 2.0, 2.0 / 3.0);
        int want = std::min(nev, K);
        for (int i = 0; i < want; ++i)
            if (std::fabs(f[i]) <= tol * std::max(eps23, std::fabs(D[i]))) ++converged;
    }
    R.converged = converged;
    if (R.positive_part) {
        int j = 0;
        while (j < K && D[j] > 0.0) ++j;
        if (j > nev) { R.pos_fail = true; return false; }
        const double scale = std::max(std::fabs(D[0]), std::fabs(D[K - 1]));
        int jn = j;
        while (jn < K && D[jn] >= -1e-12 * scale) ++jn;
        const double posres = lanczos_posres();
        if (converged >= j && (jn == K || std::fabs(f[jn]) <= std::max(tol, posres * scale))) { R.pos_count = j; return false; }
        if (K < krylovdim || R.numiter == R.maxiter) { R.pos_fail = true; return false; }
    } else {
        if (converged >= R.howmany) return false;
        if (K < krylovdim) return false;
    }
    if (R.numiter == R.maxiter) return false;
    const int keep = R.arpack ? std::min(krylovdim - 1, nev + std::max(1, (krylovdim - nev) / 2))
                              : (3 * krylovdim + 2 * converged) / 5;
    lz_restart(W, R, K, keep, speculated);
    return true;
}

inline void Solver::lz_rayleigh(EigWork& W, LzRun& R, int K, double betaK, bool from_arrow, bool check_first) {
    std::vector<double>& D = R.D; std::vector<double>& U = R.U; std::vector<double>& f = R.f;
    if (K == 1) {
        D[0] = R.T[0]; U.assign(1, 1.0); f[0] = betaK;
        return;
    }
    R.Tw.assign((size_t)K * K, 0.0);
    for (int c = 0; c < K; ++c)
        for (int r = 0; r < K; ++r) R.Tw[(size_t)c * K + r] = R.T[(size_t)c * R.ld + r];
    std::vector<double> Dasc(K);
    const double te0 = now_s();
    if (from_arrow && R.m_arrow > 0 && K > R.m_arrow)
        symeig_tridiag_from(K, R.m_arrow, R.Qa.data(), R.da.data(), R.ea.data(), R.al.data(), R.be.data(), R.Tw.data(), Dasc.data());
    else
        symeig_dense(K, R.Tw.data(), Dasc.data(), check_first);
    W.lst.host_eig_time += now_s() - te0; W.lst.host_eigs++;
    U.assign((size_t)K * K, 0.0);
    for (int c = 0; c < K; ++c) {
        D[c] = Dasc[K - 1 - c];
        for (int r = 0; r < K; ++r) U[(size_t)c * K + r] = R.Tw[(size_t)(K - 1 - c) * K + r];
        f[c] = betaK * U[(size_t)c * K + (K - 1)];
    }
}

inline void Solver::lz_restart(EigWork& W, LzRun& R, int K, int keep, bool speculated) {
    const std::vector<double>& D = R.D; const std::vector<double>& f = R.f;
    if (!R.wide) for (int j = 0; j < keep; ++j) { W.arrow_host.p[j] = f[j]; W.arrow_host.p[dev::MAXK + j] = D[j]; }
    if (R.merge_active) lz_merge_vectors(W, R, keep);
    rotate(W, K, R.U, K, keep, W.Z.p, K, keep, W.arrow_host.p, R.wide ? 0 : 2 * dev::MAXK);
    std::swap(W.V.p, W.Z.p);
    std::fill(R.T.begin(), R.T.end(), 0.0);
    const int ld = R.ld;
    for (int j = 0; j < keep; ++j) {
        R.T[(size_t)j * ld + j] = D[j];
        R.T[(size_t)j * ld + keep] = f[j];
        R.T[(size_t)keep * ld + j] = f[j];
    }
    R.kfirst = keep;
    R.presymv = speculated;
    ++R.numiter;
    W.lst.lanczos_restarts++;
}

inline void Solver::lz_finish_run(EigWork& W, LzRun& R) {
    const int K = R.K, nev = R.nev;
    W.numiter = R.numiter;
    if (R.positive_part) {
        if (R.pos_fail || R.pos_count < 0) { W.converged = false; return; }
        W.count = R.pos_count; W.converged_eigs = R.pos_count; W.converged = true;
        W.vals.assign(R.D.begin(), R.D.begin() + R.pos_count);
        if (R.pos_count > 0 && R.merge_active) lz_merge_vectors(W, R, R.pos_count);
        if (R.pos_count > 0) rotate(W, K, R.U, K, R.pos_count, W.Z.p, -1, 0, nullptr, 0);
        return;
    }
    if (R.pos_fail) { W.converged = false; return; }
    if (R.arpack) {
        W.converged_eigs = R.converged;
        if (R.converged < nev) { W.converged = false; return; }
        W.count = nev;
        W.vals.assign(R.D.begin(), R.D.begin() + nev);
        std::reverse(W.vals.begin(), W.vals.end());
        std::vector<double> Ur((size_t)K * nev);
        for (int c = 0; c < nev; ++c)
            for (int r = 0; r < K; ++r) Ur[(size_t)c * K + r] = R.U[(size_t)(nev - 1 - c) * K + r];
        rotate(W, K, Ur, K, nev, W.Z.p, -1, 0, nullptr, 0);
        W.converged = true;
        return;
    }
    int howmany = R.howmany;
    if (R.converged > howmany) howmany = R.converged;
    W.count = howmany;
    W.vals.assign(R.D.begin(), R.D.begin() + howmany);
    W.converged_eigs = R.converged;
    W.converged = (R.converged != 0);
    if (R.merge_active) lz_merge_vectors(W, R, howmany);
    rotate(W, K, R.U, K, howmany, W.Z.p, -1, 0, nullptr, 0);
}

inline void Solver::lanczos_eager(EigWork& W, const double* xp, int nev) {
    LzRun& R = W.lzrun;
    W.use_fop = false;
    if (!lz_init(W, R, nev, false)) return;
    if (R.arpack) throw std::invalid_argument("krylovkit_eager applies to eigsolver = 2 (KrylovKit) only");
    if (R.wide) throw std::invalid_argument("krylovkit_eager: Krylov dimension > 255 is not supported");
    const int kd = R.krylovdim, ld = R.ld;
    const double tol = R.tol;
    lz_launch_begin(W, W.resid.p, W.ctl_p);
    std::vector<double>& T = R.T; std::vector<double>& f = R.f;
    std::vector<double> fstep(2 * dev::MAXK, 0.0);
    int K = 0, kfirst = 0, converged = 0;
    double beta = 0.0;
    while (true) {
        const int k = K;
        launch_symv(W, xp, W.V.p + (size_t)k * W.npad, true);
        int keep = kfirst;
        if (k > kfirst) {
            std::fill(fstep.begin(), fstep.begin() + k, 0.0);
            fstep[k - 1] = beta;
            W.arrow.upload(fstep.data(), (size_t)k, stream);
            W.arrow_p = W.arrow.p;
            keep = k;
        }
        with_nch(k + 1, [&](auto nch) {
            auto kern = dev::k_lz_orth<decltype(nch)::value, 0>;
            hipLaunchKernelGGL(kern, dim3(W.nt), dim3(dev::TPB), 0, stream,
                               (const double*)W.Ppart.p, W.nt, W.npad, (const double*)W.V.p, W.npad, k, W.w.p,
                               (const double*)W.hred.p, lz_hpart(W, k), W.pld, W.hsum1.p, (const dev::LanczosCtl*)W.ctl_p,
                               (const double*)W.alphas_p, (const double*)W.betas_p, (const double*)W.Apart.p, W.napart, 1,
                               (const double*)W.arrow_p, keep, dev::FopArgs{});
        });
        lz_launch_finish(W, k, 0.0, false);
        PX_HIP(hipMemcpyAsync(W.rec_host, W.rec.p, EigWork::REC_DOUBLES * sizeof(double), hipMemcpyDeviceToHost, stream));
        PX_HIP(hipStreamSynchronize(stream));
        const double al_k = W.rec_host[k];
        beta = W.rec_host[dev::MAXK + k];
        W.lst.lanczos_matvecs++; W.mv_iter++;
        if (!(beta == beta) || !(al_k == al_k)) { R.pos_fail = true; R.K = K; break; }
        T[(size_t)k * ld + k] = al_k;
        if (k > kfirst) { T[(size_t)(k - 1) * ld + k] = T[(size_t)k * ld + (k - 1)] = W.rec_host[dev::MAXK + k - 1]; }
        K = k + 1;
        if (beta <= tol && K < R.howmany) R.howmany = K;
        if (K == kd || beta <= tol || K >= R.howmany) {
            lz_rayleigh(W, R, K, beta, false, false);
            converged = 0;
            while (converged < K && std::fabs(f[converged]) <= tol) ++converged;
            R.K = K; R.converged = converged;
            if (converged >= R.howmany) break;
        }
        if (K < kd) {
            if (beta <= tol) { R.K = K; break; }
            continue;
        }
        if (R.numiter == R.maxiter) break;
        lz_restart(W, R, K, (3 * kd + 2 * converged) / 5, false);
        kfirst = K = R.kfirst;
    }
    lz_finish_run(W, R);
}

inline bool Solver::lz_split_first(EigWork& W, LzRun& R, int k1) {
    R.split_ready = false;
    R.m_arrow = 0;
    if (hipEventSynchronize(W.ev_early) != hipSuccess) return false;
    const double t0 = now_s();
    const double* al_e = W.rec_early.p;
    const double* be_e = W.rec_early.p + dev::MAXK;
    dev::LanczosCtl c{};
    std::memcpy(&c, W.rec_early.p + 2 * dev::MAXK, sizeof(c));
    const int m = R.kfirst;
    bool ok = !c.stop;
    for (int j = m; ok && j < k1; ++j) ok = (al_e[j] == al_e[j]) && (be_e[j] == be_e[j]) && be_e[j] > 0.0;
    if (ok) {
        std::vector<double> Dk(std::max(m, 1)), fk(std::max(m, 1));
        for (int j = 0; j < m; ++j) { Dk[j] = R.T[(size_t)j * R.ld + j]; fk[j] = R.T[(size_t)j * R.ld + m]; }
        ok = R.split_ref().first(k1, m, Dk.data(), fk.data(), al_e, be_e) == 0;
    }
    R.split_ready = ok;
    W.lst.host_eig_overlap_time += now_s() - t0;
    return ok;
}

inline void Solver::lz_launch_step(EigWork& W, const double* xp, int k, int kfirst, double step_tol, bool& presymv) {
    if (k == kfirst) {
        if (!presymv) launch_symv(W, xp, W.V.p + (size_t)k * W.npad, true);
        else count_matvecs(W, 1);
        presymv = false;
    } else {
        launch_symv_finish(W, xp, k - 1, step_tol, k - 1 > kfirst);
    }
    dev::FopArgs fo{};
    if (W.use_fop) {
        fo.Vp = W.F.p + (size_t)W.F_first * W.npad; fo.lam = W.Flam.p; fo.rp = W.F_r;
        fo.tpart = W.tpart.p; fo.ebuf = W.ebuf.p; fo.apart = W.apartf.p;
    }
    const bool prof_o = opt.profile_symv_every > 0 && (W.lst.symv_launches % opt.profile_symv_every) == 1;
    hipEvent_t e0 = nullptr, e1 = nullptr;
    if (prof_o) std::tie(e0, e1) = W.evo.acquire();
    auto launch_orth = [&](auto kern) {
        launch_prof(prof_o, e0, e1, kern, dim3(W.nt), stream,
                    (const double*)W.Ppart.p, W.nt, W.npad, (const double*)W.V.p, W.npad, k, W.w.p,
                    (const double*)W.hred.p, lz_hpart(W, k), W.pld, W.hsum1.p,
                    (const dev::LanczosCtl*)W.ctl_p, (const double*)W.alphas_p, (const double*)W.betas_p,
                    (const double*)W.Apart.p, W.napart, k == kfirst ? 1 : 0, (const double*)W.arrow_p,
                    kfirst, fo);
    };
    with_nch(k + 1, [&](auto nch) {
        constexpr int NCH = decltype(nch)::value;
        if (!W.use_fop) launch_orth(dev::k_lz_orth<NCH, 0>);
        else if (W.F_r <= 64) launch_orth(dev::k_lz_orth<NCH, 1>);
        else launch_orth(dev::k_lz_orth<NCH, 2>);
    });
}

inline bool Solver::lanczos_certificate(EigWork& W, const double* xp, int npos, int msteps, double& theta_max, double& scale) {
    if (npos + msteps + 1 > W.cap || npos + msteps + 1 > dev::KLD || msteps < 2) return false;
    if (W.resid2.n == 0) {
        std::vector<double> r2(W.npad, 0.0);
        start_vector(W.n, (uint64_t)opt.eigsolver_resid_seed ^ 0x9e3779b97f4a7c15ull, 3, r2.data());
        W.resid2.alloc(W.npad);
        W.resid2.upload(r2.data(), W.npad, stream);
        PX_HIP(hipStreamSynchronize(stream));
    }
    std::swap(W.V.p, W.Z.p);
    if (npos == 0) {
        lz_launch_begin(W, W.resid2.p, W.ctl_p);
    } else {
        PX_HIP(hipMemcpyAsync(W.w.p, W.resid2.p, (size_t)W.npad * sizeof(double), hipMemcpyDeviceToDevice, stream));
        const int kc = npos - 1;
        with_nch(npos, [&](auto nch) {
            hipLaunchKernelGGL(dev::k_lz_measure<decltype(nch)::value>, dim3(W.nt), dim3(dev::TPB), 0, stream,
                               (const double*)W.w.p, (const double*)W.V.p, W.npad, kc, lz_hpart(W, kc), W.pld, W.ctl_p);
        });
        lz_launch_finish(W, kc, 0.0, false);
    }
    for (int j = 0; j < npos; ++j) { W.arrow_host.p[j] = 0.0; W.arrow_host.p[dev::MAXK + j] = W.vals[j]; }
    if (npos > 0) {
        PX_HIP(hipMemcpyAsync(W.arrow.p, W.arrow_host.p, (size_t)npos * sizeof(double), hipMemcpyHostToDevice, stream));
        PX_HIP(hipMemcpyAsync(W.arrow.p + dev::MAXK, W.arrow_host.p + dev::MAXK, (size_t)npos * sizeof(double), hipMemcpyHostToDevice, stream));
    }
    W.arrow_p = W.arrow.p;
    const int kend = npos + msteps;
    bool presymv = false;
    for (int k = npos; k < kend; ++k) lz_launch_step(W, xp, k, npos, 0.0, presymv);
    lz_launch_finish(W, kend - 1, 0.0, kend - 1 > npos);
    PX_HIP(hipMemcpyAsync(W.rec_host, W.rec.p, EigWork::REC_DOUBLES * sizeof(double), hipMemcpyDeviceToHost, stream));
    wait_stream();
    std::swap(W.V.p, W.Z.p);
    W.evo.used = 0; W.ev.used = 0;
    W.lst.lanczos_matvecs += msteps; W.mv_iter += msteps; W.lst.cert_matvecs += msteps;
    dev::LanczosCtl hctl{};
    std::memcpy(&hctl, W.rec_host + 2 * dev::MAXK, sizeof(hctl));
    if (hctl.stop) msteps = std::max(0, std::min(msteps, hctl.kstop - npos));
    if (msteps < 1) return false;
    const double* al = W.rec_host + npos;
    const double* be = W.rec_host + dev::MAXK + npos;
    std::vector<double> T((size_t)msteps * msteps, 0.0), d(msteps, 0.0);
    for (int j = 0; j < msteps; ++j) {
        if (!(al[j] == al[j]) || !(j + 1 < msteps ? be[j] == be[j] : true)) return false;
        T[(size_t)j * msteps + j] = al[j];
        if (j + 1 < msteps) T[(size_t)j * msteps + j + 1] = T[(size_t)(j + 1) * msteps + j] = be[j];
    }
    if (msteps == 1) d[0] = al[0];
    else if (symeig_dense(msteps, T.data(), d.data(), true) != 0) return false;
    theta_max = d[msteps - 1];
    scale = std::max({std::fabs(d[0]), std::fabs(theta_max), npos > 0 ? std::fabs(W.vals[0]) : 0.0});
    return true;
}

inline void Solver::lanczos(EigWork& W, const double* xp, int nev, bool positive_part) {
    W.ritz_ok = false;
    if (opt.krylovkit_eager && opt.eigsolver != 1 && !positive_part) { lanczos_eager(W, xp, nev); return; }
    LzRun& R = W.lzrun;
    if (!lz_init(W, R, nev, positive_part)) return;
    const int krylovdim = R.krylovdim;
    const double step_tol = R.step_tol;
    const bool wide = R.wide;
    if (wide) W.lst.wide_krylov_projections++;
    if (krylovdim >= 96) QlPool::get().arm();
    dev::LanczosCtl* const ctl = wide ? W.ctlw_p : W.ctl_p;
    const bool warm_start = positive_part ? (opt.lanczos_warm_start >= 0) : (opt.lanczos_warm_start > 0);
    if (!wide && warm_start && W.fop_ok && W.have_factors && W.F_r > 0 && W.tpart.n > 0) {
        const int nb = ceil_div(W.npad, dev::TPB);
        hipLaunchKernelGGL(dev::k_lz_warm_sum, dim3(nb), dim3(dev::TPB), 0, stream,
                           W.V.p, (const double*)(W.F.p + (size_t)W.F_first * W.npad), W.npad, W.F_r,
                           (const double*)W.resid.p, W.npad, W.warm_part.p,
                           (const double*)(positive_part && W.F_r <= dev::TPB ? W.Flam.p : nullptr),
                           positive_part ? opt.full_eig_lanczos_warm_pow : 0.0);
        hipLaunchKernelGGL(dev::k_lz_warm_scale, dim3(nb), dim3(dev::TPB), 0, stream,
                           W.V.p, W.npad, (const double*)W.warm_part.p, nb, W.ctl_p);
        W.lst.warm_starts++;
    } else
        lz_launch_begin(W, W.resid.p, ctl);

    const int merge_from = opt.host_eig_merge == 0 ? (1 << 30) : (opt.host_eig_merge == 1 ? 24 : 64);
    const bool blk1 = !wide && block1_plan(W, krylovdim, !R.arpack && krylovdim >= merge_from);
    const bool use_split = !wide && !blk1 && !R.arpack && krylovdim >= merge_from;
    struct PoolGuard { SpinPool* p; ~PoolGuard() { if (p) p->disarm(); } } pool_guard{nullptr};
    W.split.M.par = nullptr;
    if (use_split && merge_helpers() > 0 && StreamRef::tl == nullptr) {
        if (!merge_pool) {
            merge_pool.reset(new SpinPool(merge_helpers()));
            merge_par = [this](int n, const std::function<void(int)>& body) { merge_pool->run(n, body); };
        }
        merge_pool->arm();
        pool_guard.p = merge_pool.get();
        W.split.M.par = &merge_par;
        W.split.M.nchunk = merge_helpers() + 1;
    }
    if (use_split && W.side == nullptr) {
        W.side.create(hipStreamNonBlocking);
        W.ev_mid.create(hipEventDisableTiming);
        W.ev_early.create(hipEventDisableTiming);
        W.rec_early.alloc(EigWork::REC_DOUBLES);
    }
    struct DeferGuard {
        EigWork& W;
        DeferGuard(EigWork& w, bool on) : W(w) { W.b1_defer = on; }
        ~DeferGuard() { W.b1_defer = false; }
    };
    while (true) {
        const int kfirst = R.kfirst;
        const int k1 = (kfirst == 0) ? (18 * krylovdim) / 25 : kfirst + 1;
        const bool split_cycle = use_split && k1 >= 1 && k1 <= krylovdim - 2;
        if (wide) {
            for (int k = kfirst; k < krylovdim; ++k) lzw_step(W, xp, k, kfirst, step_tol, R.presymv);
        } else if (blk1) {
            launch_block1(W, xp, kfirst, krylovdim, step_tol);
            R.presymv = false;
        } else {
            for (int k = kfirst; k < krylovdim; ++k) {
                lz_launch_step(W, xp, k, kfirst, step_tol, R.presymv);
                if (split_cycle && k == k1) {
                    PX_HIP(hipEventRecord(W.ev_mid, stream));
                    PX_HIP(hipStreamWaitEvent(W.side, W.ev_mid, 0));
                    PX_HIP(hipMemcpyAsync(W.rec_early.p, W.rec.p, EigWork::REC_DOUBLES * sizeof(double), hipMemcpyDeviceToHost, W.side));
                    PX_HIP(hipEventRecord(W.ev_early, W.side));
                }
            }
            lz_launch_finish(W, krylovdim - 1, step_tol, krylovdim - 1 > kfirst);
        }
        const bool speculate = !blk1 && (W.prev_numiter > 1 || R.numiter > 1);
        if (speculate) {
            launch_symv(W, xp, W.V.p + (size_t)krylovdim * W.npad, true, ctl);
            count_matvecs(W, -1);
        }
        if (wide) PX_HIP(hipMemcpyAsync(W.recw_pinned.p, W.recw.p, EigWork::RECW_DOUBLES * sizeof(double), hipMemcpyDeviceToHost, stream));
        else PX_HIP(hipMemcpyAsync(W.rec_host, W.rec.p, EigWork::REC_DOUBLES * sizeof(double), hipMemcpyDeviceToHost, stream));
        if (!(split_cycle && lz_split_first(W, R, k1))) lz_prepare_arrow(R);
        const double tdbg0 = debug ? now_s() : 0.0;
        wait_stream();
        if (debug) { dbg_lz[0] += now_s() - tdbg0; dbg_lz[5] += 1.0; }
        if (W.cye_pending) {
            W.cye_pending = false;
            float ms = 0.f;
            if (hipEventElapsedTime(&ms, W.cye[0], W.cye[1]) == hipSuccess) W.lst.cycle_ms += ms;
        }
        W.ev.harvest(W.lst.symv_profiled_ms, W.lst.symv_profiled);
        W.evo.harvest(W.lst.orth_profiled_ms, W.lst.orth_profiled);
        const double tdbg1 = debug ? now_s() : 0.0;
        bool go_on;
        {
            DeferGuard defer(W, blk1);
            go_on = lz_after_cycle(W, R, speculate);
        }
        if (debug) dbg_lz[1] += now_s() - tdbg1;
        if (!go_on) break;
    }
    const double tdbg2 = debug ? now_s() : 0.0;
    lz_finish_run(W, R);
    if (debug) dbg_lz[3] += now_s() - tdbg2;
}

inline void Solver::lzw_step(EigWork& W, const double* xp, int k, int kfirst, double step_tol, bool& presymv) {
    if (k == kfirst && presymv) {
        count_matvecs(W, 1);
    } else {
        launch_symv(W, xp, W.V.p + (size_t)k * W.npad, true, W.ctlw_p);
    }
    presymv = false;
    const dev::LanczosCtl* ctl = W.ctlw_p;
    const int nred = ceil_div(k + 2, dev::TPB);
    hipLaunchKernelGGL(dev::k_lzw_dots, dim3(W.nt), dim3(dev::TPB), 0, stream,
                       (const double*)W.Ppart.p, W.nt, W.npad, (const double*)W.V.p, W.npad, k, W.w.p, W.hpw1.p, ctl);
    hipLaunchKernelGGL(dev::k_lzw_reduce, dim3(nred), dim3(dev::TPB), 0, stream,
                       (const double*)W.hpw1.p, W.pld, W.nt, k, W.hsw1.p, ctl, 0);
    hipLaunchKernelGGL(dev::k_lzw_update, dim3(W.nt), dim3(dev::TPB), 0, stream,
                       W.w.p, (const double*)W.V.p, W.npad, k, (const double*)W.hsw1.p, W.hpw2.p, W.pld, ctl);
    hipLaunchKernelGGL(dev::k_lzw_reduce, dim3(nred), dim3(dev::TPB), 0, stream,
                       (const double*)W.hpw2.p, W.pld, W.nt, k, W.hsw2.p, ctl, 1);
    hipLaunchKernelGGL(dev::k_lzw_close, dim3(W.nt), dim3(dev::TPB), 0, stream,
                       (const double*)W.w.p, W.V.p, W.npad, k, (const double*)W.hsw1.p, (const double*)W.hsw2.p,
// ... 402 lines not shown
        mask_d.alloc(t.mask_words); mask_d.upload(t.mask, t.mask_words, stream);
        P.blocks.assign(1, BlockInfo{n, N, t.mask_off});
        tile_base.assign(1, 0);
        rstride = grid;
        filled(respart_d, (size_t)2 * grid);
    }
    const double* sc = t.use_dsc ? dsc.p : nullptr;
    switch (t.epilogue) {
        case 0: sym_gemm<dev::SG_PLAIN, false>(W, dP.p, dQ.p, dT.p, nullptr, t.ca, t.cb, t.cc, sc, dpart.p, nullptr, nullptr, -1); break;
        case 1: sym_gemm<dev::SG_POLY, false>(W, dP.p, dQ.p, dT.p, dY.p, t.ca, t.cb, t.cc, sc, dpart.p, nullptr, nullptr, -1); break;
        case 2: sym_gemm<dev::SG_FINAL, false>(W, dP.p, dQ.p, nullptr, nullptr, t.ca, t.cb, t.cc, sc, dpart.p, dxp.p, nullptr, -1); break;
        default: sym_gemm<dev::SG_FINAL, true>(W, dP.p, dQ.p, nullptr, nullptr, t.ca, t.cb, t.cc, sc, dpart.p, dxp.p, dxold.p, 0); break;
    }
    PX_HIP(hipGetLastError());
    if (!fin) dT.download(t.T, sz, stream);
    if (t.part) dpart.download(t.part, grid, stream);
    if (fin) dxp.download(t.xp, N, stream);
    if (fuse) respart_d.download(t.respart, (size_t)2 * grid, stream);
    PX_HIP(hipStreamSynchronize(stream));
    t.ld = ld;
    t.grid = grid;
}

inline void Solver::test_sign_unpack(const double* packed, double sentinel, double* A, double* sc) {
    EigWork& W = eig[0];
    const int ld = W.nt * dev::TILE;
    const size_t sz = (size_t)ld * ld;
    DevBuf<double> xp(W.N), As(sz), dsc(16);
    xp.upload(packed, W.N, stream);
    std::vector<double> h(sz, sentinel);
    As.upload(h.data(), sz, stream);
    W.sgA.alloc(sz); W.sgY.alloc(sz);
    W.sgA.zero(stream); W.sgY.zero(stream);
    W.sg_ld = ld;
    sign_choose_tiles(W);
    W.sg_part.alloc(W.sg_npart);
    dsc.zero(stream);
    sign_unpack(W, xp.p, As.p, dsc.p);
    sign_unpack(W, xp.p, W.sgA.p, dsc.p);
    sign_scale(W, dsc.p);
    PX_HIP(hipGetLastError());
    As.download(A, sz, stream);
    dsc.download(sc, 16, stream);
    PX_HIP(hipStreamSynchronize(stream));
}

inline void Solver::run_blocks(const std::vector<int>& blocks, const std::function<void(int)>& job) {
    bool have_streams = true;
    for (int idx : blocks) have_streams = have_streams && eig[idx].stream != nullptr;
    if (!parallel_blocks() || blocks.size() < 2 || !have_streams) {
        for (int idx : blocks) job(idx);
        merge_block_stats();
        return;
    }
    PX_HIP(hipEventRecord(ev_main, stream.main));
    block_pool->run(blocks, [this, &job](int idx) {
        struct TlReset { ~TlReset() { StreamRef::tl = nullptr; } } reset;
        StreamRef::tl = eig[idx].stream;
        PX_HIP(hipStreamWaitEvent(eig[idx].stream, ev_main, 0));
        job(idx);
        PX_HIP(hipEventRecord(eig[idx].done, eig[idx].stream));
    });
    for (int idx : blocks) PX_HIP(hipStreamWaitEvent(stream.main, eig[idx].done, 0));
    merge_block_stats();
}
inline void Solver::merge_block_stats() {
#define PX_MERGE(f) st.f += a.f
    for (EigWork& W : eig) {
        proxsdp_stats& a = W.lst;
        PX_MERGE(lanczos_matvecs); PX_MERGE(lanczos_restarts); PX_MERGE(lanczos_calls);
        PX_MERGE(full_eigs); PX_MERGE(krylov_fallbacks);
        PX_MERGE(symv_launches); PX_MERGE(symv_bytes);
        PX_MERGE(symv_profiled); PX_MERGE(symv_profiled_ms);
        PX_MERGE(orth_profiled); PX_MERGE(orth_profiled_ms);
        PX_MERGE(full_eig_solver_ms); PX_MERGE(full_eig_recon_ms);
        PX_MERGE(full_eigs_lanczos); PX_MERGE(full_eigs_lanczos_checks); PX_MERGE(full_eigs_lanczos_mismatches);
        PX_MERGE(full_eigs_lanczos_certified); PX_MERGE(full_eigs_lanczos_cert_failed); PX_MERGE(cert_matvecs);
        PX_MERGE(dense_truncated_projections); PX_MERGE(wide_krylov_projections);
        PX_MERGE(full_eigs_sign); PX_MERGE(sign_products); PX_MERGE(sign_short_pass); PX_MERGE(sign_short_fail);
        PX_MERGE(sign_engine_projections); PX_MERGE(sign_engine_rejected);
        PX_MERGE(sign_engine_checks); PX_MERGE(sign_engine_mismatches);
        PX_MERGE(batched_block_steps);
        PX_MERGE(host_eigs); PX_MERGE(host_eig_time); PX_MERGE(host_eig_merges); PX_MERGE(host_eig_overlap_time);
        PX_MERGE(warm_starts); PX_MERGE(device_eigs); PX_MERGE(mfma_reconstructions);
        PX_MERGE(cycle_launches); PX_MERGE(cycle_steps); PX_MERGE(cycle_ms);
        PX_MERGE(fop_projections);
        a = proxsdp_stats{};
        lz_matvec_iter += W.mv_iter; recon_r_iter += W.recon_r;
        W.mv_iter = 0; W.recon_r = 0;
    }
#undef PX_MERGE
}

}
```

Measured before the change: 534.0.

## Move split Lanczos rank-one eigen-merge onto the GPU and rotate from device vectors

Adds a device kernel path (DeviceMerge) for the divide-and-conquer rank-one merge of the split tridiagonal eigenproblem. The first half is staged on a side stream, and the merged eigenvectors stay on the GPU so the Ritz rotation reads them directly. This removes the host secular-equation solve, the host Qf rotation and the eigenvector upload. It is on by default when krylovdim >= 64 and K <= 255, and falls back to the host merge otherwise. The risks are extra GPU launches on the critical path and numerical differences from the host solver.

```diff
diff --git a/include/proxsdp_hip.h b/include/proxsdp_hip.h
--- a/include/proxsdp_hip.h
+++ b/include/proxsdp_hip.h
@@ -135,7 +135,8 @@
     int32_t reserved_i3[2];
     int32_t block_batch_groups;
     int32_t lanczos_wide_krylov;
-    int32_t reserved_i2[7];
+    int32_t reserved_i2[6];
+    int32_t device_eig_merge;
     double  full_eig_lanczos_warm_pow;
     double  reserved_d2[3];
 } proxsdp_options;
@@ -201,6 +202,8 @@
     int64_t dense_sigma_steps;
 } proxsdp_stats;
 #define PROXSDP_STATS_SHARDED_GENERAL_ITERATIONS 0
+#define PROXSDP_STATS_DEVICE_EIG_MERGES 1
+#define PROXSDP_STATS_DEVICE_EIG_MERGE_FALLBACKS 2
 
 typedef struct proxsdp_result {
     int32_t status;
@@ -421,6 +424,11 @@
                               const double* al, const double* be, double* U, double* d, int32_t* info);
 int proxsdp_host_symeig_split_threads(int32_t K, int32_t m, int32_t k1, const double* D, const double* f,
                                       const double* al, const double* be, int32_t threads, double* U, double* d, int32_t* info);
+int proxsdp_device_symeig_split(int32_t K, int32_t m, int32_t k1, const double* D, const double* f,
+                                const double* al, const double* be, double* U, double* d, int32_t* info);
+int proxsdp_host_merge_plan(int32_t K, int32_t m, int32_t k1, const double* D, const double* f, const double* al,
+                            const double* be, int32_t with_qf, double* Q1, double* Q2, double* Qf, double* d, double* z,
+                            int32_t* colsrc, int32_t* nd, int32_t* rot_idx, double* rot_cs, int32_t* counts);
 int proxsdp_host_start_vector(int64_t n, int64_t seed, int32_t init, double* out);
 int proxsdp_host_preprocess(const proxsdp_problem* prob, int64_t* order, int64_t* var_ordering,
                             double* c_scaled, double* frobenius_norm_M);
diff --git a/proxsdp.jl_amd/binding.py b/proxsdp.jl_amd/binding.py
--- a/proxsdp.jl_amd/binding.py
+++ b/proxsdp.jl_amd/binding.py
@@ -101,7 +101,7 @@
     a("sign_start_row", i32); a("general_batch", i32); a("full_eig_lanczos_certify", i32); a("host_merge_threads", i32); a("reserved_i", i32 * 1)
     a("full_eig_lanczos_tol", f64); a("reserved_d", f64 * 1)
     a("equilibration_reference_aliasing", i32); a("reserved_i3", i32 * 2)
-    a("block_batch_groups", i32); a("lanczos_wide_krylov", i32); a("reserved_i2", i32 * 7); a("full_eig_lanczos_warm_pow", f64); a("reserved_d2", f64 * 3)
+    a("block_batch_groups", i32); a("lanczos_wide_krylov", i32); a("reserved_i2", i32 * 6); a("device_eig_merge", i32); a("full_eig_lanczos_warm_pow", f64); a("reserved_d2", f64 * 3)
     return F
 
 
@@ -143,7 +143,7 @@
                 ("status_string", C.c_char * 256), ("stats", Stats)]
 
 
-STATS_RESERVED_SLOTS = {"sharded_general_iterations": 0}
+STATS_RESERVED_SLOTS = {"sharded_general_iterations": 0, "device_eig_merges": 1, "device_eig_merge_fallbacks": 2}
 
 STATE_NHIST = 7
 STATE_HIST_NAMES = ("dual_gap", "prim_obj", "dual_obj", "feasibility", "primal_residual", "dual_residual", "comb_residual")
@@ -1088,6 +1088,43 @@
     return d, U.T.copy(), dict(nondeflated=info[0], deflated=info[1], max_secular_iterations=info[2])
 
 
+def device_symeig_split(D, f, al, be, k1):
+    D = _f(D); f = _f(f); al = _f(al); be = _f(be)
+    K, m = len(al), len(D)
+    U = np.zeros((K, K))
+    d = np.zeros(K)
+    info = (i32 * 3)()
+    L = lib()
+    L.proxsdp_device_symeig_split.argtypes = [i32, i32, i32, pf64, pf64, pf64, pf64, pf64, pf64, C.POINTER(i32)]
+    L.proxsdp_device_symeig_split.restype = C.c_int
+    _check(L.proxsdp_device_symeig_split(K, m, int(k1), _p(D) if m else None, _p(f) if m else None, _p(al), _p(be),
+                                         _p(U), _p(d), info))
+    return d, U.T.copy(), dict(nondeflated=info[0], deflated=info[1], max_secular_iterations=info[2])
+
+
+def host_merge_plan(D, f, al, be, k1, with_qf):
+    D = _f(D); f = _f(f); al = _f(al); be = _f(be)
+    K, m = len(al), len(D)
+    k1 = int(k1); k2 = K - k1
+    Q1 = np.zeros((k1, k1)); Q2 = np.zeros((k2, k2)); Qf = np.zeros((K, K))
+    d = np.zeros(K); z = np.zeros(K)
+    colsrc = np.zeros(K, dtype=np.int32); nd = np.zeros(K, dtype=np.int32)
+    ridx = np.zeros(2 * K, dtype=np.int32); rcs = np.zeros(2 * K)
+    counts = (i32 * 3)()
+    pi32 = C.POINTER(i32)
+    L = lib()
+    L.proxsdp_host_merge_plan.argtypes = [i32, i32, i32, pf64, pf64, pf64, pf64, i32, pf64, pf64, pf64, pf64, pf64,
+                                          pi32, pi32, pi32, pf64, pi32]
+    L.proxsdp_host_merge_plan.restype = C.c_int
+    _check(L.proxsdp_host_merge_plan(K, m, k1, _p(D) if m else None, _p(f) if m else None, _p(al), _p(be), int(bool(with_qf)),
+                                     _p(Q1), _p(Q2), _p(Qf), _p(d), _p(z), colsrc.ctypes.data_as(pi32), nd.ctypes.data_as(pi32),
+                                     ridx.ctypes.data_as(pi32), _p(rcs), counts))
+    k, ndf, nrot = counts[0], counts[1], counts[2]
+    rots = [(int(ridx[2 * q]), int(ridx[2 * q + 1]), float(rcs[2 * q]), float(rcs[2 * q + 1])) for q in range(nrot)]
+    return dict(Q1=Q1.T.copy(), Q2=Q2.T.copy(), Qf=Qf.T.copy() if with_qf else None, d=d, z=z, colsrc=colsrc.copy(),
+                nd=nd[:k].copy(), rots=rots, deflated=ndf)
+
+
 def host_preprocess(prob, index_base=0):
     M = _Marshalled(prob, index_base=index_base)
     n = prob.n
diff --git a/proxsdp.jl_amd/csrc/capi.hip b/proxsdp.jl_amd/csrc/capi.hip
--- a/proxsdp.jl_amd/csrc/capi.hip
+++ b/proxsdp.jl_amd/csrc/capi.hip
@@ -959,6 +959,61 @@
         return 0;
     });
 }
+int proxsdp_device_symeig_split(int32_t K, int32_t m, int32_t k1, const double* D, const double* f,
+                                const double* al, const double* be, double* U, double* d, int32_t* info) {
+    return guarded([&]() -> int {
+        if (K < 2 || m < 0 || m >= K || k1 < 1 || k1 >= K || !al || !be || !U || !d) throw std::invalid_argument("invalid argument");
+        if (!proxsdp::DeviceMerge::eligible(K)) throw std::invalid_argument("device merge serves 2 <= K <= 255");
+        proxsdp::SplitEig S;
+        if (S.first(k1, m, D, f, al, be) != 0 || S.tail(K, al, be) != 0) throw std::invalid_argument("split eigensolver failed");
+        proxsdp::DeviceMerge dm;
+        proxsdp::Stream st;
+        st.create(hipStreamNonBlocking);
+        dm.stage_first(S, st);
+        std::vector<double> Dd(K), fd(K);
+        const bool ok = dm.run(S, K, 1.0, st, [](hipEvent_t e) { PX_HIP(hipEventSynchronize(e)); }, Dd.data(), fd.data());
+        std::vector<double> Ud((size_t)K * K);
+        std::vector<int> it(std::max(dm.k, 1), 0);
+        dm.Uall.download(Ud.data(), Ud.size(), st);
+        if (dm.k > 0) dm.iters_d.download(it.data(), (size_t)dm.k, st);
+        PX_HIP(hipStreamSynchronize(st));
+        if (!ok) throw std::runtime_error("device merge handed the eigensolve back");
+        for (int c = 0; c < K; ++c) {
+            d[c] = Dd[K - 1 - c];
+            std::copy(Ud.begin() + (size_t)(K - 1 - c) * K, Ud.begin() + (size_t)(K - c) * K, U + (size_t)c * K);
+        }
+        if (info) { info[0] = dm.k; info[1] = dm.ndf; info[2] = dm.k > 0 ? *std::max_element(it.begin(), it.end()) : 0; }
+        return 0;
+    });
+}
+
+int proxsdp_host_merge_plan(int32_t K, int32_t m, int32_t k1, const double* D, const double* f, const double* al,
+                            const double* be, int32_t with_qf, double* Q1, double* Q2, double* Qf, double* d, double* z,
+                            int32_t* colsrc, int32_t* nd, int32_t* rot_idx, double* rot_cs, int32_t* counts) {
+    return guarded([&]() -> int {
+        if (K < 2 || m < 0 || m >= K || k1 < 1 || k1 >= K || !al || !be || !Q1 || !Q2 || !Qf || !d || !z || !colsrc || !nd ||
+            !rot_idx || !rot_cs || !counts) throw std::invalid_argument("invalid argument");
+        proxsdp::SplitEig S;
+        if (S.first(k1, m, D, f, al, be) != 0 || S.tail(K, al, be) != 0) throw std::invalid_argument("split eigensolver failed");
+        const int k2 = K - k1;
+        proxsdp::Rank1Merge& M = S.M;
+        M.plan(k1, k2, S.Q1.data(), S.d1.data(), S.Q2.data(), S.d2.data(), S.beta, with_qf != 0);
+        std::copy(S.Q1.begin(), S.Q1.end(), Q1);
+        std::copy(S.Q2.begin(), S.Q2.end(), Q2);
+        if (with_qf) std::copy(M.Qf.begin(), M.Qf.end(), Qf);
+        std::copy(M.d.begin(), M.d.end(), d);
+        std::copy(M.z.begin(), M.z.end(), z);
+        std::copy(M.colsrc.begin(), M.colsrc.end(), colsrc);
+        std::copy(M.nd.begin(), M.nd.end(), nd);
+        for (size_t q = 0; q < M.rots.size(); ++q) {
+            rot_idx[2 * q] = M.rots[q].pj; rot_idx[2 * q + 1] = M.rots[q].j;
+            rot_cs[2 * q] = M.rots[q].c; rot_cs[2 * q + 1] = M.rots[q].s;
+        }
+        counts[0] = M.k; counts[1] = (int)M.df.size(); counts[2] = (int)M.rots.size();
+        return 0;
+    });
+}
+
 int proxsdp_host_start_vector(int64_t n, int64_t seed, int32_t init, double* out) {
     if (n < 0 || !out) { g_last_error = "invalid argument"; return PROXSDP_E_INVALID; }
     proxsdp::start_vector(n, (uint64_t)seed, init, out);
diff --git a/proxsdp.jl_amd/csrc/host_eig_merge.hpp b/proxsdp.jl_amd/csrc/host_eig_merge.hpp
--- a/proxsdp.jl_amd/csrc/host_eig_merge.hpp
+++ b/proxsdp.jl_amd/csrc/host_eig_merge.hpp
@@ -34,6 +34,15 @@
     if (u3) { _mm256_storeu_pd(u3, a03); _mm256_storeu_pd(u3 + 4, a13); }
 }
 #endif
+
+static inline bool rank1_panel_uses_fma() {
+#if defined(__x86_64__)
+    static const bool have_fma = __builtin_cpu_supports("avx2") && __builtin_cpu_supports("fma");
+    return have_fma;
+#else
+    return false;
+#endif
+}
 
 using ParFor = std::function<void(int, const std::function<void(int)>&)>;
 
@@ -135,25 +144,36 @@
     }
 
     void build(int k1_, int k2_, const double* Q1, const double* d1, const double* Q2, const double* d2, double beta) {
+        plan(k1_, k2_, Q1, d1, Q2, d2, beta, true);
+        solve();
+    }
+
+    struct Rot { int pj, j; double c, s; };
+    std::vector<int> colsrc;
+    std::vector<Rot> rots;
+    void plan(int k1_, int k2_, const double* Q1, const double* d1, const double* Q2, const double* d2, double beta, bool with_Qf) {
         const double eps = 2.220446049250313e-16;
         k1 = k1_; k2 = k2_; K = k1 + k2;
         const double sgn = beta < 0.0 ? -1.0 : 1.0;
         rho = 2.0 * std::fabs(beta);
         const double isq2 = 0.70710678118654752440;
         d.assign(K, 0.0); z.assign(K, 0.0); ctype.assign(K, 0);
-        Qf.assign((size_t)K * K, 0.0);
+        colsrc.assign(K, 0); rots.clear();
+        if (with_Qf) Qf.assign((size_t)K * K, 0.0);
         {
             int a = 0, b = 0;
             for (int p = 0; p < K; ++p) {
                 const bool takeA = (b >= k2) || (a < k1 && d1[a] <= d2[b]);
-                double* col = Qf.data() + (size_t)p * K;
+                double* col = with_Qf ? Qf.data() + (size_t)p * K : nullptr;
                 if (takeA) {
                     d[p] = d1[a]; z[p] = Q1[(size_t)a * k1 + (k1 - 1)] * isq2; ctype[p] = 1;
-                    for (int r = 0; r < k1; ++r) col[r] = Q1[(size_t)a * k1 + r];
+                    colsrc[p] = a;
+                    if (with_Qf) for (int r = 0; r < k1; ++r) col[r] = Q1[(size_t)a * k1 + r];
                     ++a;
                 } else {
                     d[p] = d2[b]; z[p] = sgn * Q2[(size_t)b * k2] * isq2; ctype[p] = 2;
-                    for (int r = 0; r < k2; ++r) col[k1 + r] = Q2[(size_t)b * k2 + r];
+                    colsrc[p] = -(b + 1);
+                    if (with_Qf) for (int r = 0; r < k2; ++r) col[k1 + r] = Q2[(size_t)b * k2 + r];
                     ++b;
                 }
             }
@@ -175,12 +195,15 @@
                 c /= tau; s = -s / tau;
                 if (std::fabs(t * c * s) <= tol) {
                     z[j] = tau; z[pj] = 0.0;
-                    double* __restrict__ x = Qf.data() + (size_t)pj * K;
-                    double* __restrict__ y = Qf.data() + (size_t)j * K;
-                    for (int r = 0; r < K; ++r) {
-                        const double xr = x[r], yr = y[r];
-                        x[r] = c * xr + s * yr;
-                        y[r] = c * yr - s * xr;
+                    rots.push_back(Rot{pj, j, c, s});
+                    if (with_Qf) {
+                        double* __restrict__ x = Qf.data() + (size_t)pj * K;
+                        double* __restrict__ y = Qf.data() + (size_t)j * K;
+                        for (int r = 0; r < K; ++r) {
+                            const double xr = x[r], yr = y[r];
+                            x[r] = c * xr + s * yr;
+                            y[r] = c * yr - s * xr;
+                        }
                     }
                     const double tt = d[pj] * c * c + d[j] * s * s;
                     d[j] = d[pj] * s * s + d[j] * c * c;
@@ -200,6 +223,9 @@
         for (int j = 0; j < k; ++j) { dn[j] = d[nd[j]]; zn[j] = z[nd[j]]; }
         for (int j = 1; j < k; ++j)
             if (!(dn[j] > dn[j - 1])) dn[j] = std::nextafter(dn[j - 1], 1e300);
+    }
+
+    void solve() {
         lam.assign(k, 0.0);
         delta.assign((size_t)k * k, 0.0);
         max_iter_seen = 0;
@@ -303,7 +329,7 @@
                 const double* w0 = wbuf.data(); const double* w1 = w0 + kk; const double* w2 = w1 + kk; const double* w3 = w2 + kk;
                 int r = 0;
 #if defined(__x86_64__)
-                static const bool have_fma = __builtin_cpu_supports("avx2") && __builtin_cpu_supports("fma");
+                const bool have_fma = rank1_panel_uses_fma();
                 for (; have_fma && r + 8 <= nr; r += 8)
                     rank1_panel_8x4(Qf.data(), K, qcol.data(), kk, r0 + r, w0, w1, w2, w3, u[0] ? u[0] + r : nullptr,
                                     u[1] ? u[1] + r : nullptr, u[2] ? u[2] + r : nullptr, u[3] ? u[3] + r : nullptr);
diff --git a/proxsdp.jl_amd/csrc/host_util.hpp b/proxsdp.jl_amd/csrc/host_util.hpp
--- a/proxsdp.jl_amd/csrc/host_util.hpp
+++ b/proxsdp.jl_amd/csrc/host_util.hpp
@@ -487,6 +487,12 @@
         return rc;
     }
     int second(int K_, const double* al, const double* be) {
+        if (tail(K_, al, be) != 0) return 1;
+        merge_host();
+        return 0;
+    }
+    void merge_host() { M.build(k1, K - k1, Q1.data(), d1.data(), Q2.data(), d2.data(), beta); }
+    int tail(int K_, const double* al, const double* be) {
         K = K_;
         const int k2 = K - k1;
         if (!have_first || k2 < 1) return 1;
@@ -496,9 +502,7 @@
             if (j + 1 < k2) { Q2[(size_t)j * k2 + j + 1] = be[k1 + j]; Q2[(size_t)(j + 1) * k2 + j] = be[k1 + j]; }
         }
         Q2[0] -= std::fabs(beta);
-        if (symeig_dense(k2, Q2.data(), d2.data(), true, 0) != 0) return 1;
-        M.build(k1, k2, Q1.data(), d1.data(), Q2.data(), d2.data(), beta);
-        return 0;
+        return symeig_dense(k2, Q2.data(), d2.data(), true, 0) != 0 ? 1 : 0;
     }
 };
 
@@ -552,7 +556,7 @@
         PX_OPT(rocsolver_warmup, OT_I32), PX_OPT(debug_fail_iteration, OT_I32), PX_OPT(host_wait_spin, OT_I32), PX_OPT(sign_start_row, OT_I32), PX_OPT(general_batch, OT_I32),
         PX_OPT(full_eig_lanczos_certify, OT_I32), PX_OPT(full_eig_lanczos_tol, OT_F64), PX_OPT(host_merge_threads, OT_I32),
         PX_OPT(equilibration_reference_aliasing, OT_I32), PX_OPT(block_batch_groups, OT_I32), PX_OPT(full_eig_lanczos_warm_pow, OT_F64),
-        PX_OPT(lanczos_wide_krylov, OT_I32),
+        PX_OPT(lanczos_wide_krylov, OT_I32), PX_OPT(device_eig_merge, OT_I32),
     };
     return t;
 }
@@ -597,7 +601,7 @@
     o->host_eig_merge = -1; o->block_batch = -1; o->rocsolver_warmup = 0; o->host_wait_spin = -1; o->sign_start_row = -1; o->general_batch = -1;
     o->full_eig_lanczos_certify = -1; o->full_eig_lanczos_tol = 0.0; o->host_merge_threads = -1;
     o->equilibration_reference_aliasing = 1; o->block_batch_groups = -1; o->full_eig_lanczos_warm_pow = 1.0;
-    o->lanczos_wide_krylov = 0;
+    o->lanczos_wide_krylov = 0; o->device_eig_merge = -1;
 }
 
 inline int set_option(proxsdp_options* o, const char* name, double v) {
diff --git a/proxsdp.jl_amd/csrc/merge_device.hip.hpp b/proxsdp.jl_amd/csrc/merge_device.hip.hpp
--- /dev/null
+++ b/proxsdp.jl_amd/csrc/merge_device.hip.hpp
@@ -0,0 +1,406 @@
+#pragma once
+
+namespace proxsdp {
+namespace dev {
+
+constexpr int MG_KMAX = 255;
+constexpr int MG_LD = 256;
+constexpr int MG_I_COLSRC = 8, MG_I_ND = MG_I_COLSRC + MG_LD, MG_I_DF = MG_I_ND + MG_LD, MG_I_RPJ = MG_I_DF + MG_LD,
+              MG_I_RJ = MG_I_RPJ + MG_LD, MG_NINT = MG_I_RJ + MG_LD;
+constexpr int MG_SC = MG_NINT / 2, MG_D = MG_SC + 2, MG_DN = MG_D + MG_LD, MG_ZN = MG_DN + MG_LD, MG_RC = MG_ZN + MG_LD,
+              MG_RS = MG_RC + MG_LD, MG_Q2 = MG_RS + MG_LD, MG_PACK = MG_Q2 + (MG_KMAX - 1) * (MG_KMAX - 1);
+static_assert(MG_NINT % 2 == 0, "the int part of the pack ends on a double");
+constexpr int MG_REC = 2 * MAXK + 8;
+constexpr double MG_TINY = 2.2250738585072014e-308;
+
+__device__ __forceinline__ void mg_stage_sync() {
+    asm volatile("s_waitcnt lgkmcnt(0)" ::: "memory");
+    __builtin_amdgcn_wave_barrier();
+}
+template <int L>
+__device__ __forceinline__ double mg_from_lane(double v) {
+    const int lo = __builtin_amdgcn_readlane(__double2loint(v), L);
+    const int hi = __builtin_amdgcn_readlane(__double2hiint(v), L);
+    return __hiloint2double(hi, lo);
+}
+__device__ __forceinline__ double mg_serial_sum(const double* st, int lo, int hi) {
+#pragma clang fp contract(off)
+    double a = 0.0;
+#pragma unroll 8
+    for (int j = lo; j < hi; ++j) a += st[j];
+    return a;
+}
+__device__ __forceinline__ int mg_wave_count(int v) { return (int)wave_sum((double)v); }
+
+__device__ __forceinline__ void mg_assemble_column(const double* __restrict__ pack, const double* __restrict__ Q1,
+                                                   double* __restrict__ Qf, int p) {
+    const int* hi = reinterpret_cast<const int*>(pack);
+    const int K = hi[0], k1 = hi[1], k2 = hi[2];
+    const int cs = hi[MG_I_COLSRC + p];
+    const double* src = cs >= 0 ? Q1 + (size_t)cs * k1 : pack + MG_Q2 + (size_t)(-(cs + 1)) * k2;
+    for (int r = threadIdx.x; r < K; r += blockDim.x) {
+        double v = 0.0;
+        if (cs >= 0) { if (r < k1) v = src[r]; }
+        else if (r >= k1) v = src[r - k1];
+        Qf[(size_t)p * K + r] = v;
+    }
+}
+
+__global__ __launch_bounds__(64) void k_mg_rotate(const double* __restrict__ pack, double* __restrict__ Qf) {
+#pragma clang fp contract(off)
+    const int* hi = reinterpret_cast<const int*>(pack);
+    const int K = hi[0], nrot = hi[5];
+    const int r = blockIdx.x * 64 + threadIdx.x;
+    if (r >= K) return;
+    for (int q = 0; q < nrot; ++q) {
+        const int pj = hi[MG_I_RPJ + q], j = hi[MG_I_RJ + q];
+        const double c = pack[MG_RC + q], s = pack[MG_RS + q];
+        const double xr = Qf[(size_t)pj * K + r], yr = Qf[(size_t)j * K + r];
+        Qf[(size_t)pj * K + r] = c * xr + s * yr;
+        Qf[(size_t)j * K + r] = c * yr - s * xr;
+    }
+}
+
+__device__ __forceinline__ void mg_eval(const double (&dnl)[4], const double (&znl)[4], int lane, int k, double dorg, double tau,
+                                        int isplit, double rho, double* sp, double* sq, double& psi, double& dpsi, double& phi,
+                                        double& dphi) {
+#pragma clang fp contract(off)
+#pragma unroll
+    for (int q = 0; q < 4; ++q) {
+        const int j = lane + 64 * q;
+        if (j < k) {
+            const double dl = (dnl[q] - dorg) - tau;
+            const double t = znl[q] / dl;
+            sp[j] = znl[q] * t; sq[j] = t * t;
+        }
+    }
+    mg_stage_sync();
+    double acc = 0.0;
+    if (lane < 4) acc = mg_serial_sum((lane & 1) ? sq : sp, lane < 2 ? 0 : isplit + 1, lane < 2 ? isplit + 1 : k);
+    mg_stage_sync();
+    psi = rho * mg_from_lane<0>(acc); dpsi = rho * mg_from_lane<1>(acc);
+    phi = rho * mg_from_lane<2>(acc); dphi = rho * mg_from_lane<3>(acc);
+}
+
+__global__ __launch_bounds__(256) void k_mg_roots(const double* __restrict__ pack, const double* __restrict__ Q1,
+                                                  double* __restrict__ Qf, double* __restrict__ lam,
+                                                  double* __restrict__ delta, int* __restrict__ iters) {
+#pragma clang fp contract(off)
+    const int* hi = reinterpret_cast<const int*>(pack);
+    const int k = hi[3];
+    const int nrb = (k + 3) >> 2;
+    if ((int)blockIdx.x >= nrb) {
+        if ((int)blockIdx.x - nrb < hi[0]) mg_assemble_column(pack, Q1, Qf, (int)blockIdx.x - nrb);
+        return;
+    }
+    __shared__ double s_st[4][2][MG_LD];
+    const int lane = threadIdx.x & 63;
+    const int i = blockIdx.x * 4 + (threadIdx.x >> 6);
+    if (i >= k) return;
+    double* sp = s_st[threadIdx.x >> 6][0];
+    double* sq = s_st[threadIdx.x >> 6][1];
+    const double* dn = pack + MG_DN;
+    const double* zn = pack + MG_ZN;
+    const double rho = pack[MG_SC];
+    const double eps = 2.220446049250313e-16;
+    double dnl[4], znl[4];
+#pragma unroll
+    for (int q = 0; q < 4; ++q) {
+        const int j = lane + 64 * q;
+        dnl[q] = j < k ? dn[j] : 0.0;
+        znl[q] = j < k ? zn[j] : 0.0;
+    }
+    int org = 0, it = 0;
+    double tau;
+    if (k == 1) {
+        tau = rho * zn[0] * zn[0];
+    } else {
+        const bool last = (i == k - 1);
+        const int ia = last ? k - 2 : i, ib = ia + 1;
+        const int isplit = ia;
+        double lo, hi_, psi, dpsi, phi, dphi;
+        if (!last) {
+            const double gap = dn[i + 1] - dn[i];
+            mg_eval(dnl, znl, lane, k, dn[i], 0.5 * gap, isplit, rho, sp, sq, psi, dpsi, phi, dphi);
+            const double fmid = 1.0 + psi + phi;
+            if (fmid >= 0.0) { org = i; lo = 0.0; hi_ = 0.5 * gap; }
+            else { org = i + 1; lo = -0.5 * gap; hi_ = 0.0; }
+        } else {
+#pragma unroll
+            for (int q = 0; q < 4; ++q)
+                if (lane + 64 * q < k) sp[lane + 64 * q] = znl[q] * znl[q];
+            mg_stage_sync();
+            double zz = lane == 0 ? mg_serial_sum(sp, 0, k) : 0.0;
+            mg_stage_sync();
+            zz = mg_from_lane<0>(zz);
+            org = k - 1; lo = 0.0; hi_ = rho * zz;
+        }
+        const double dorg = dn[org];
+        const double dia = dn[ia] - dorg, dib = dn[ib] - dorg;
+        tau = 0.5 * (lo + hi_);
+        double f = 0.0;
+        for (; it < 80; ++it) {
+            if (!(tau > lo && tau < hi_)) tau = 0.5 * (lo + hi_);
+            if (tau == lo || tau == hi_) break;
+            mg_eval(dnl, znl, lane, k, dorg, tau, isplit, rho, sp, sq, psi, dpsi, phi, dphi);
+            f = 1.0 + psi + phi;
+            const double erretm = 8.0 * (fabs(psi) + fabs(phi)) + 2.0 + fabs(tau) * (dpsi + dphi);
+            if (fabs(f) <= eps * erretm) break;
+            if (f < 0.0) lo = tau; else hi_ = tau;
+            if (hi_ - lo <= 2.0 * eps * fmax(fabs(lo), fabs(hi_))) { tau = 0.5 * (lo + hi_); break; }
+            const double Da = dia - tau, Db = dib - tau;
+            const double s = dpsi * Da * Da, Sb = dphi * Db * Db;
+            const double c = f - dpsi * Da - dphi * Db;
+            const double bq = c * (Da + Db) + s + Sb;
+            const double w = Da * Db * f;
+            double eta;
+            if (c == 0.0) {
+                eta = (bq != 0.0) ? w / bq : 0.0;
+            } else {
+                double disc = bq * bq - 4.0 * c * w;
+                if (disc < 0.0) disc = 0.0;
+                const double sq = sqrt(disc);
+                const double qq = (bq >= 0.0) ? 0.5 * (bq + sq) : 0.5 * (bq - sq);
+                const double e1 = (qq != 0.0) ? w / qq : 0.0;
+                const double e2 = qq / c;
+                const double t1 = tau + e1, t2 = tau + e2;
+                const bool in1 = (t1 > lo && t1 < hi_), in2 = (t2 > lo && t2 < hi_);
+                if (in1 && in2) eta = (fabs(e1) <= fabs(e2)) ? e1 : e2;
+                else if (in1) eta = e1;
+                else if (in2) eta = e2;
+                else eta = 0.5 * (lo + hi_) - tau;
+            }
+            double tn = tau + eta;
+            if (!(tn > lo && tn < hi_) || !(tn == tn)) tn = 0.5 * (lo + hi_);
+            if (tn == tau) break;
+            tau = tn;
+        }
+    }
+    const double dorg = dn[org];
+    const double lm = dorg + tau;
+#pragma unroll
+    for (int q = 0; q < 4; ++q) {
+        const int j = lane + 64 * q;
+        if (j < k) {
+            double dl = (dnl[q] - dorg) - tau;
+            if (j == i && dl >= 0.0) dl = -MG_TINY;
+            if (j == i + 1 && dl <= 0.0) dl = MG_TINY;
+            delta[(size_t)i * k + j] = dl;
+        }
+    }
+    if (lane == 0) { lam[i] = lm; iters[i] = it; }
+}
+
+__global__ __launch_bounds__(256) void k_mg_weights(const double* __restrict__ pack, const double* __restrict__ delta,
+                                                    double* __restrict__ zhat) {
+#pragma clang fp contract(off)
+    const int* hi = reinterpret_cast<const int*>(pack);
+    const int k = hi[3];
+    __shared__ double s_st[4][MG_LD];
+    const int lane = threadIdx.x & 63;
+    const int j = blockIdx.x * 4 + (threadIdx.x >> 6);
+    if (j >= k) return;
+    double* st = s_st[threadIdx.x >> 6];
+    const double* dn = pack + MG_DN;
+    const double rho = pack[MG_SC];
+    const double dj = dn[j];
+#pragma unroll
+    for (int q = 0; q < 4; ++q) {
+        const int i = lane + 64 * q;
+        if (i < k - 1) st[i] = delta[(size_t)i * k + j] / (dj - dn[i < j ? i : i + 1]);
+    }
+    mg_stage_sync();
+    if (lane == 0) {
+        double prod = -delta[(size_t)(k - 1) * k + j];
+#pragma unroll 8
+        for (int i = 0; i < k - 1; ++i) prod *= st[i];
+        const double v = sqrt(fabs(prod) / rho);
+        zhat[j] = pack[MG_ZN + j] < 0.0 ? -v : v;
+    }
+}
+
+__global__ __launch_bounds__(256) void k_mg_vectors(const double* __restrict__ pack, const double* __restrict__ Qf,
+                                                    const double* __restrict__ lam, const double* __restrict__ delta,
+                                                    const double* __restrict__ zhat, const int* __restrict__ iters,
+                                                    double* __restrict__ S, double* __restrict__ rec, int* __restrict__ src) {
+#pragma clang fp contract(off)
+    const int* hi = reinterpret_cast<const int*>(pack);
+    const int K = hi[0], k = hi[3];
+    __shared__ double s_st[4][MG_LD];
+    const int lane = threadIdx.x & 63;
+    const int t = blockIdx.x * 4 + (threadIdx.x >> 6);
+    if (t >= K) return;
+    double* st = s_st[threadIdx.x >> 6];
+    const int* nd = hi + MG_I_ND;
+    const int* df = hi + MG_I_DF;
+    const double* d = pack + MG_D;
+    double v, e;
+    if (t < k) {
+        double s[4];
+#pragma unroll
+        for (int q = 0; q < 4; ++q) {
+            const int j = lane + 64 * q;
+            s[q] = j < k ? zhat[j] / delta[(size_t)t * k + j] : 0.0;
+            if (j < k) st[j] = s[q] * s[q];
+        }
+        mg_stage_sync();
+        double nn = lane == 0 ? mg_serial_sum(st, 0, k) : 0.0;
+        mg_stage_sync();
+        nn = mg_from_lane<0>(nn);
+        const double inv = 1.0 / sqrt(nn);
+#pragma unroll
+        for (int q = 0; q < 4; ++q) {
+            const int j = lane + 64 * q;
+            if (j < k) {
+                s[q] *= inv;
+                S[(size_t)t * k + j] = s[q];
+                st[j] = Qf[(size_t)nd[j] * K + (K - 1)] * s[q];
+            }
+        }
+        mg_stage_sync();
+        e = lane == 0 ? mg_serial_sum(st, 0, k) : 0.0;
+        mg_stage_sync();
+        e = mg_from_lane<0>(e);
+        v = lam[t];
+    } else {
+        const int p = df[t - k];
+        v = d[p];
+        e = Qf[(size_t)p * K + (K - 1)];
+    }
+    int cnt = 0;
+    for (int u = lane; u < K; u += 64) {
+        const double vu = u < k ? lam[u] : d[df[u - k]];
+        cnt += (vu < v || (vu == v && u < t)) ? 1 : 0;
+    }
+    cnt = mg_wave_count(cnt);
+    if (lane == 0) {
+        const int c = K - 1 - cnt;
+        rec[c] = pack[MG_SC + 1] * e;
+        rec[MAXK + c] = v;
+        src[c] = t;
+    }
+    if (t == 0) {
+        int bad = 0;
+        for (int u = lane; u < k; u += 64) bad += (iters[u] >= 80 || !(fabs(lam[u]) <= 1.7976931348623157e308)) ? 1 : 0;
+        bad = mg_wave_count(bad);
+        if (lane == 0) rec[2 * MAXK] = (double)bad;
+    }
+}
+
+__global__ __launch_bounds__(256) void k_mg_eigvecs(const double* __restrict__ pack, const double* __restrict__ Qf,
+                                                    const double* __restrict__ S, const int* __restrict__ src,
+                                                    double* __restrict__ Uall) {
+#pragma clang fp contract(off)
+    __shared__ double s_s[MG_LD];
+    __shared__ int s_nd[MG_LD];
+    const int* hi = reinterpret_cast<const int*>(pack);
+    const int K = hi[0], k = hi[3];
+    const int c = blockIdx.x, r = threadIdx.x;
+    const int t = src[c];
+    if (t >= k) {
+        if (r < K) Uall[(size_t)c * K + r] = Qf[(size_t)hi[MG_I_DF + (t - k)] * K + r];
+        return;
+    }
+    if (r < k) { s_s[r] = S[(size_t)t * k + r]; s_nd[r] = hi[MG_I_ND + r]; }
+    __syncthreads();
+    if (r >= K) return;
+    const int k1 = hi[1], k2 = hi[2];
+    const bool fused = hi[6] != 0 && (r < k1 ? r < (k1 & ~7) : r - k1 < (k2 & ~7));
+    double acc = 0.0;
+    int j = 0;
+    for (; j + 8 <= k; j += 8) {
+        double q[8];
+#pragma unroll
+        for (int u = 0; u < 8; ++u) q[u] = Qf[(size_t)s_nd[j + u] * K + r];
+        if (fused) {
+#pragma unroll
+            for (int u = 0; u < 8; ++u) acc = fma(q[u], s_s[j + u], acc);
+        } else {
+#pragma unroll
+            for (int u = 0; u < 8; ++u) acc += q[u] * s_s[j + u];
+        }
+    }
+    for (; j < k; ++j) {
+        const double q = Qf[(size_t)s_nd[j] * K + r];
+        if (fused) acc = fma(q, s_s[j], acc); else acc += q * s_s[j];
+    }
+    Uall[(size_t)c * K + r] = acc;
+}
+
+}
+
+struct DeviceMerge {
+    DevBuf<double> Q1d, pack_d, Qf, lam, delta, zhat, S, rec_d, Uall;
+    DevBuf<int> iters_d, src_d;
+    PinnedBuf q1_h, pack_h, rec_h;
+    Event ev_q1, ev_rec;
+    bool ready = false;
+    int K = 0, k = 0, ndf = 0;
+    void ensure() {
+        if (ready) return;
+        const size_t kk = (size_t)dev::MG_KMAX * dev::MG_KMAX;
+        Q1d.alloc(kk); pack_d.alloc(dev::MG_PACK); Qf.alloc(kk); lam.alloc(dev::MG_LD); delta.alloc(kk); zhat.alloc(dev::MG_LD);
+        S.alloc(kk); rec_d.alloc(dev::MG_REC); Uall.alloc(kk);
+        iters_d.alloc(dev::MG_LD); src_d.alloc(dev::MG_LD);
+        q1_h.alloc(kk); pack_h.alloc(dev::MG_PACK); rec_h.alloc(dev::MG_REC);
+        ev_q1.create(hipEventDisableTiming); ev_rec.create(hipEventDisableTiming);
+        ready = true;
+    }
+    static bool eligible(int K) { return K >= 2 && K <= dev::MG_KMAX; }
+    void stage_first(const SplitEig& Sp, hipStream_t side) {
+        ensure();
+        const size_t n1 = (size_t)Sp.k1 * Sp.k1;
+        if (Sp.k1 < 1 || Sp.k1 >= dev::MG_KMAX) throw std::logic_error("device merge: first part too large");
+        std::memcpy(q1_h.p, Sp.Q1.data(), n1 * sizeof(double));
+        PX_HIP(hipMemcpyAsync(Q1d.p, q1_h.p, n1 * sizeof(double), hipMemcpyHostToDevice, side));
+        PX_HIP(hipEventRecord(ev_q1, side));
+    }
+    template <typename Wait>
+    bool run(SplitEig& Sp, int K_, double betaK, hipStream_t stream, Wait&& wait, double* D, double* f) {
+        ensure();
+        Rank1Merge& M = Sp.M;
+        const int k1 = Sp.k1, k2 = K_ - k1;
+        if (!eligible(K_) || k1 < 1 || k2 < 1) return false;
+        M.plan(k1, k2, Sp.Q1.data(), Sp.d1.data(), Sp.Q2.data(), Sp.d2.data(), Sp.beta, false);
+        K = K_; k = M.k; ndf = (int)M.df.size();
+        const int nrot = (int)M.rots.size();
+        if (k + ndf != K || nrot >= dev::MG_LD) throw std::logic_error("device merge: inconsistent plan");
+        int* hi = reinterpret_cast<int*>(pack_h.p);
+        hi[0] = K; hi[1] = k1; hi[2] = k2; hi[3] = k; hi[4] = ndf; hi[5] = nrot; hi[6] = rank1_panel_uses_fma() ? 1 : 0; hi[7] = 0;
+        for (int p = 0; p < K; ++p) hi[dev::MG_I_COLSRC + p] = M.colsrc[p];
+        for (int j = 0; j < k; ++j) hi[dev::MG_I_ND + j] = M.nd[j];
+        for (int j = 0; j < ndf; ++j) hi[dev::MG_I_DF + j] = M.df[j];
+        double* pd = pack_h.p;
+        pd[dev::MG_SC] = M.rho; pd[dev::MG_SC + 1] = betaK;
+        for (int q = 0; q < nrot; ++q) {
+            hi[dev::MG_I_RPJ + q] = M.rots[q].pj; hi[dev::MG_I_RJ + q] = M.rots[q].j;
+            pd[dev::MG_RC + q] = M.rots[q].c; pd[dev::MG_RS + q] = M.rots[q].s;
+        }
+        for (int p = 0; p < K; ++p) pd[dev::MG_D + p] = M.d[p];
+        for (int j = 0; j < k; ++j) { pd[dev::MG_DN + j] = M.dn[j]; pd[dev::MG_ZN + j] = M.zn[j]; }
+        std::memcpy(pd + dev::MG_Q2, Sp.Q2.data(), (size_t)k2 * k2 * sizeof(double));
+        PX_HIP(hipMemcpyAsync(pack_d.p, pack_h.p, ((size_t)dev::MG_Q2 + (size_t)k2 * k2) * sizeof(double), hipMemcpyHostToDevice, stream));
+        PX_HIP(hipStreamWaitEvent(stream, ev_q1, 0));
+        const double* pk = pack_d.p;
+        hipLaunchKernelGGL(dev::k_mg_roots, dim3((k + 3) / 4 + K), dim3(256), 0, stream, pk, (const double*)Q1d.p, Qf.p, lam.p,
+                           delta.p, iters_d.p);
+        if (nrot > 0) hipLaunchKernelGGL(dev::k_mg_rotate, dim3((K + 63) / 64), dim3(64), 0, stream, pk, Qf.p);
+        if (k > 0) hipLaunchKernelGGL(dev::k_mg_weights, dim3((k + 3) / 4), dim3(256), 0, stream, pk, (const double*)delta.p, zhat.p);
+        hipLaunchKernelGGL(dev::k_mg_vectors, dim3((K + 3) / 4), dim3(256), 0, stream, pk, (const double*)Qf.p, (const double*)lam.p,
+                           (const double*)delta.p, (const double*)zhat.p, (const int*)iters_d.p, S.p, rec_d.p, src_d.p);
+        PX_HIP(hipMemcpyAsync(rec_h.p, rec_d.p, dev::MG_REC * sizeof(double), hipMemcpyDeviceToHost, stream));
+        PX_HIP(hipEventRecord(ev_rec, stream));
+        hipLaunchKernelGGL(dev::k_mg_eigvecs, dim3(K), dim3(256), 0, stream, pk, (const double*)Qf.p, (const double*)S.p,
+                           (const int*)src_d.p, Uall.p);
+        PX_HIP(hipGetLastError());
+        wait((hipEvent_t)ev_rec);
+        const double* r = rec_h.p;
+        bool ok = (r[2 * dev::MAXK] == 0.0);
+        for (int c = 0; ok && c < K; ++c) ok = std::isfinite(r[c]) && std::isfinite(r[dev::MAXK + c]);
+        if (!ok) return false;
+        for (int c = 0; c < K; ++c) { f[c] = r[c]; D[c] = r[dev::MAXK + c]; }
+        return true;
+    }
+};
+
+}
diff --git a/proxsdp.jl_amd/csrc/solver.hip.hpp b/proxsdp.jl_amd/csrc/solver.hip.hpp
--- a/proxsdp.jl_amd/csrc/solver.hip.hpp
+++ b/proxsdp.jl_amd/csrc/solver.hip.hpp
@@ -159,6 +159,7 @@
 }
 }
 #include "shard_comm.hip.hpp"
+#include "merge_device.hip.hpp"
 namespace proxsdp {
 
 struct CircularVector {
@@ -216,6 +217,10 @@
     SplitEig& split_ref() { return *splitp; }
     bool split_ready = false;
     bool merge_active = false;
+    bool dev_wanted = false;
+    bool dev_merge = false;
+    bool dev_staged = false;
+    bool merge_on_device = false;
     std::vector<double> erow;
 };
 
@@ -265,6 +270,7 @@
     int ritz_first = 0, ritz_r = 0;
     PinnedBuf rec_early;
     SplitEig split;
+    DeviceMerge dmerge;
     int batch_slot = 0;
     bool b1_defer = false;
     int b1_rot_K = 0;
@@ -439,6 +445,7 @@
     void extract_factors(const std::vector<double>& x);
     void rotate(EigWork& W, int K, const std::vector<double>& U, int ldu, int ncols, double* out, int copy_src, int copy_dst,
                 const double* extra, int nextra);
+    void rotate_launch(EigWork& W, int K, const double* Ud, int ncols, double* out, int copy_src, int copy_dst);
 
     void test_project(int idx, double* xp, int tr);
     void test_full_eig(const double* xin, double* xout) { current_rank.assign(1, 0); min_eig.assign(1, 0.0); full_eig_project(0, xin, xout, false); }
@@ -986,10 +993,14 @@
     }
     W.U.upload(tmp, (size_t)K * ncols + (size_t)std::max(nextra, 0), stream);
     if (nextra > 0) W.arrow_p = W.U.p + (size_t)K * ncols;
+    rotate_launch(W, K, W.U.p, ncols, out, copy_src, copy_dst);
+}
+
+inline void Solver::rotate_launch(EigWork& W, int K, const double* Ud, int ncols, double* out, int copy_src, int copy_dst) {
     if (W.lzrun.wide) {
         if (ncols > 0 || copy_src >= 0)
             hipLaunchKernelGGL(dev::k_lzw_rotate, dim3(W.nt, std::max(1, ceil_div(ncols, dev::LZW_RC))), dim3(dev::TPB), 0, stream,
-                               (const double*)W.V.p, W.npad, K, (const double*)W.U.p, ncols, out, W.npad, copy_src, copy_dst);
+                               (const double*)W.V.p, W.npad, K, Ud, ncols, out, W.npad, copy_src, copy_dst);
         return;
     }
     {
@@ -997,7 +1008,7 @@
         const size_t lds_m = ((size_t)Kp * dev::RM_LDV + (size_t)dev::RM_CG * (Kp + 2)) * sizeof(double);
         if (K >= 32 && ncols >= 16 && (int)lds_m <= rotate_mfma_lds_cap) {
             hipLaunchKernelGGL(dev::k_lz_rotate_mfma, dim3(W.nt, ceil_div(ncols, dev::RM_CG)), dim3(dev::TPB), lds_m, stream,
-                               (const double*)W.V.p, W.npad, K, (const double*)W.U.p, ncols, out, W.npad, copy_src, copy_dst);
+                               (const double*)W.V.p, W.npad, K, Ud, ncols, out, W.npad, copy_src, copy_dst);
             return;
         }
     }
@@ -1009,7 +1020,7 @@
         const bool last = (c0 + cn >= ncols);
         if (cn > 0 || (last && copy_src >= 0))
             hipLaunchKernelGGL(dev::k_lz_rotate, dim3(W.nt), dim3(dev::TPB), (size_t)K * cn * 8 + vbytes, stream,
-                               W.V.p, W.npad, W.n, K, W.U.p + (size_t)c0 * K, K, cn,
+                               W.V.p, W.npad, W.n, K, Ud + (size_t)c0 * K, K, cn,
                                out + (size_t)c0 * W.npad, W.npad, last ? copy_src : -1, copy_dst - c0);
         c0 += std::max(cn, 1);
     } while (c0 < ncols);
@@ -1043,6 +1054,7 @@
     R.howmany = nev; R.numiter = 1; R.converged = 0; R.K = 0; R.kfirst = 0; R.pos_count = -1;
     R.pos_fail = false; R.presymv = false; R.betaK = 0.0;
     R.split_ready = false; R.merge_active = false;
+    R.dev_wanted = R.dev_merge = R.dev_staged = R.merge_on_device = false;
     R.splitp = &W.split;
     return true;
 }
@@ -1093,22 +1105,37 @@
         return false;
     }
     if (betaK <= tol && K < R.howmany && !R.arpack) R.howmany = K;
-    R.merge_active = false;
+    R.merge_active = false; R.merge_on_device = false;
     if (K > 1 && R.split_ready && K == krylovdim) {
         const double te0 = now_s();
-        if (R.split_ref().second(K, al.data(), be.data()) == 0) {
-            R.erow.resize(K);
-            R.split_ref().M.row_of_vectors(K - 1, R.erow.data());
-            for (int c = 0; c < K; ++c) {
-                D[c] = R.split_ref().M.evals[K - 1 - c];
-                f[c] = betaK * R.erow[K - 1 - c];
+        double waited = 0.0;
+        SplitEig& Sp = R.split_ref();
+        if (Sp.tail(K, al.data(), be.data()) == 0) {
+            bool on_device = false;
+            if (R.dev_merge && R.dev_staged)
+                on_device = W.dmerge.run(Sp, K, betaK, stream, [&](hipEvent_t e) {
+                    const double tw0 = now_s();
+                    wait_event(e);
+                    waited = now_s() - tw0;
+                }, D.data(), f.data());
+            if (on_device) {
+                W.lst.reserved_s[PROXSDP_STATS_DEVICE_EIG_MERGES]++;
+            } else {
+                if (R.dev_wanted) W.lst.reserved_s[PROXSDP_STATS_DEVICE_EIG_MERGE_FALLBACKS]++;
+                Sp.merge_host();
+                R.erow.resize(K);
+                Sp.M.row_of_vectors(K - 1, R.erow.data());
+                for (int c = 0; c < K; ++c) {
+                    D[c] = Sp.M.evals[K - 1 - c];
+                    f[c] = betaK * R.erow[K - 1 - c];
+                }
             }
-            R.merge_active = true;
+            R.merge_active = true; R.merge_on_device = on_device;
             W.lst.host_eigs++; W.lst.host_eig_merges++;
         }
-        W.lst.host_eig_time += now_s() - te0;
-    }
-    R.split_ready = false;
+        W.lst.host_eig_time += now_s() - te0 - waited;
+    }
+    R.split_ready = false; R.dev_staged = false;
     if (!R.merge_active) lz_rayleigh(W, R, K, betaK, true, kfirst == 0);
     int converged = 0;
     if (!R.arpack) {
@@ -1170,9 +1197,14 @@
 
 inline void Solver::lz_restart(EigWork& W, LzRun& R, int K, int keep, bool speculated) {
     const std::vector<double>& D = R.D; const std::vector<double>& f = R.f;
-    if (!R.wide) for (int j = 0; j < keep; ++j) { W.arrow_host.p[j] = f[j]; W.arrow_host.p[dev::MAXK + j] = D[j]; }
-    if (R.merge_active) lz_merge_vectors(W, R, keep);
-    rotate(W, K, R.U, K, keep, W.Z.p, K, keep, W.arrow_host.p, R.wide ? 0 : 2 * dev::MAXK);
+    if (R.merge_on_device) {
+        W.arrow_p = W.dmerge.rec_d.p;
+        rotate_launch(W, K, W.dmerge.Uall.p, keep, W.Z.p, K, keep);
+    } else {
+        if (!R.wide) for (int j = 0; j < keep; ++j) { W.arrow_host.p[j] = f[j]; W.arrow_host.p[dev::MAXK + j] = D[j]; }
+        if (R.merge_active) lz_merge_vectors(W, R, keep);
+        rotate(W, K, R.U, K, keep, W.Z.p, K, keep, W.arrow_host.p, R.wide ? 0 : 2 * dev::MAXK);
+    }
     std::swap(W.V.p, W.Z.p);
     std::fill(R.T.begin(), R.T.end(), 0.0);
     const int ld = R.ld;
@@ -1194,6 +1226,7 @@
         if (R.pos_fail || R.pos_count < 0) { W.converged = false; return; }
         W.count = R.pos_count; W.converged_eigs = R.pos_count; W.converged = true;
         W.vals.assign(R.D.begin(), R.D.begin() + R.pos_count);
+        if (R.pos_count > 0 && R.merge_on_device) { rotate_launch(W, K, W.dmerge.Uall.p, R.pos_count, W.Z.p, -1, 0); return; }
         if (R.pos_count > 0 && R.merge_active) lz_merge_vectors(W, R, R.pos_count);
         if (R.pos_count > 0) rotate(W, K, R.U, K, R.pos_count, W.Z.p, -1, 0, nullptr, 0);
         return;
@@ -1218,6 +1251,7 @@
     W.vals.assign(R.D.begin(), R.D.begin() + howmany);
     W.converged_eigs = R.converged;
     W.converged = (R.converged != 0);
+    if (R.merge_on_device) { rotate_launch(W, K, W.dmerge.Uall.p, howmany, W.Z.p, -1, 0); return; }
     if (R.merge_active) lz_merge_vectors(W, R, howmany);
     rotate(W, K, R.U, K, howmany, W.Z.p, -1, 0, nullptr, 0);
 }
@@ -1301,6 +1335,8 @@
         ok = R.split_ref().first(k1, m, Dk.data(), fk.data(), al_e, be_e) == 0;
     }
     R.split_ready = ok;
+    R.dev_staged = false;
+    if (ok && R.dev_merge) { W.dmerge.stage_first(R.split_ref(), W.side); R.dev_staged = true; }
     W.lst.host_eig_overlap_time += now_s() - t0;
     return ok;
 }
@@ -1432,6 +1468,8 @@
         W.split.M.par = &merge_par;
         W.split.M.nchunk = merge_helpers() + 1;
     }
+    R.dev_wanted = use_split && (opt.device_eig_merge == 1 || (opt.device_eig_merge < 0 && krylovdim >= 64));
+    R.dev_merge = R.dev_wanted && rot_sink == nullptr && StreamRef::tl == nullptr && DeviceMerge::eligible(krylovdim);
     if (use_split && W.side == nullptr) {
         W.side.create(hipStreamNonBlocking);
         W.ev_mid.create(hipEventDisableTiming);
@@ -2000,6 +2038,7 @@
         PX_MERGE(sign_engine_checks); PX_MERGE(sign_engine_mismatches);
         PX_MERGE(batched_block_steps);
         PX_MERGE(host_eigs); PX_MERGE(host_eig_time); PX_MERGE(host_eig_merges); PX_MERGE(host_eig_overlap_time);
+        PX_MERGE(reserved_s[PROXSDP_STATS_DEVICE_EIG_MERGES]); PX_MERGE(reserved_s[PROXSDP_STATS_DEVICE_EIG_MERGE_FALLBACKS]);
         PX_MERGE(warm_starts); PX_MERGE(device_eigs); PX_MERGE(mfma_reconstructions);
         PX_MERGE(cycle_launches); PX_MERGE(cycle_steps); PX_MERGE(cycle_ms);
         PX_MERGE(fop_projections);
```

Result: faster. 553.2, median of 6 (+3.6%).
